# TimD1/vcfdist

Hardware: AMD Instinct MI355X
Metric: supercluster-alignments/sec (higher is better)
Workload: dtype int32; 1 GPU; wgs_synth; superclusters_per_gpu=1000000, span_dist=lognormal(median 20, sigma 1.2) clip [4,10000]

## Files before the change

### vcfdist_amd/csrc/pr_api.hip

```cpp
#include <hip/hip_runtime.h>
#include <hip/hip_ext.h>
#include <dlfcn.h>

#include <algorithm>
#include <atomic>
#include <chrono>
#include <cstdarg>
#include <cstdio>
#include <cstdlib>
#include <cstring>
#include <condition_variable>
#include <deque>
#include <functional>
#include <mutex>
#include <string>
#include <thread>
#include <tuple>
#include <unordered_map>
#include <unordered_set>
#include <vector>

#include "../../include/vcfdist_pr.h"
#include "pr_device.h"
#include "pr_plan.h"
extern "C" int vpr_batch_skeleton_from_variants(const vpr_variants *v, vpr_owned_batch **out);
#include "pr_kernels.hip"
#include "pr_band.hip"
#include "pr_walkseg.hip"
#include "pr_q16.hip"
#include "pr_zl.hip"
#include "pr_d1.hip"
#include "pr_ed.hip"
#include "pr_gen.hip"
#include "pr_wide.hip"
#include "pr_strip.hip"
#include "pr_tie.hip"

#include "pr_host.h"

namespace {


inline int plan_level_of(int lv, int long_lt, int Lt) { return (lv <= LV_Q16 && Lt >= long_lt) ? LONG_LV : lv; }

AlnDesc plan_desc(const vpr_handle *h, const Plan &P, size_t k) {
    if (!P.lazy) return P.descs[k];
    AlnDesc d = h->descs[size_t(P.work[k])];
    (void)window_layout(d, plan_level_of(P.lv, P.long_lt, d.Lt), int64_t(P.off128[k]) * 128, P.tag_or);
    return d;
}

__global__ void k_build_plan(BatchOffsets O, const int32_t *__restrict__ work, const uint32_t *__restrict__ off128, int n, int lv,
                             int long_lt, int tag_or, AlnDesc *__restrict__ plan_descs, AlnDesc *__restrict__ descs) {
    const int k = blockIdx.x * blockDim.x + threadIdx.x;
    if (k >= n) return;
    const int a = work[k];
    AlnDesc d = base_desc(O, a);
    const int dl = (lv <= LV_Q16 && d.Lt >= long_lt) ? 2  : lv;
    (void)window_layout(d, dl, int64_t(off128[k]) * 128, tag_or);
    plan_descs[k] = d;
    descs[a] = d;
}

__global__ void k_plan_keys(BatchOffsets O, int n_al, int lv, int long_lt, uint16_t *__restrict__ keys, int32_t *__restrict__ vals,
                            uint32_t *__restrict__ need) {
    const int a = blockIdx.x * blockDim.x + threadIdx.x;
    if (a >= n_al) return;
    const int sc = a >> 2, i = a & 3, qs = i >> 1, ts = 2 + (i & 1);
    AlnDesc d{};
    d.Lq = int32_t(O.hap_off[qs][sc + 1] - O.hap_off[qs][sc]);
    d.Lt = int32_t(O.hap_off[ts][sc + 1] - O.hap_off[ts][sc]);
    d.Lr = int32_t(O.ref_off[sc + 1] - O.ref_off[sc]);
    d.path_cap = d.Lq + d.Lr + d.Lt + 4;
    const int dl = (lv <= LV_Q16 && d.Lt >= long_lt) ? 2  : lv;
    keys[a] = d.Lt >= long_lt ? uint16_t(0xffff) : uint16_t(d.Lt);
    vals[a] = a;
    need[a] = uint32_t(window_layout(d, dl, 0, 0) / 128);
}
__global__ void k_plan_gather(const int32_t *__restrict__ order, const uint32_t *__restrict__ need, uint32_t *__restrict__ out,
                              int32_t *__restrict__ pos, int n) {
    const int k = blockIdx.x * blockDim.x + threadIdx.x;
    if (k >= n) return;
    const int a = order[k];
    out[k] = need[a];
    pos[a] = k;
}
__global__ void __launch_bounds__(64) k_zl_hdr(BatchOffsets O, const int32_t *__restrict__ order, int n_short, ZlWave *__restrict__ hdr) {
    const int w = blockIdx.x, lane = threadIdx.x;
    const int j = w * 64 + lane;
    int lq = 0, lr = 0, lt = 0;
    if (j < n_short) {
        const int a = order[j];
        const int sc = a >> 2, i = a & 3, qs = i >> 1, ts = 2 + (i & 1);
        lq = int32_t(O.hap_off[qs][sc + 1] - O.hap_off[qs][sc]);
        lt = int32_t(O.hap_off[ts][sc + 1] - O.hap_off[ts][sc]);
        lr = int32_t(O.ref_off[sc + 1] - O.ref_off[sc]);
    }
#pragma unroll
    for (int o = 32; o; o >>= 1) {
        lq = max(lq, __shfl_xor(lq, o)); lr = max(lr, __shfl_xor(lr, o)); lt = max(lt, __shfl_xor(lt, o));
    }
    if (lane == 0) {
        ZlWave W;
        W.in_off = 0; W.log_off = 0; W.mq = lq; W.mr = lr; W.mt = lt; W.pad = 0;
        hdr[w] = W;
    }
}
__global__ void __launch_bounds__(1024) k_zl_scan(ZlWave *__restrict__ hdr, int n_waves, int64_t *__restrict__ totals) {
    __shared__ int64_t s_in[1024], s_log[1024];
    __shared__ int s_len;
    const int tid = threadIdx.x;
    if (tid == 0) s_len = 0;
    const int per = (n_waves + 1023) / 1024;
    const int b = min(n_waves, tid * per), e = min(n_waves, b + per);
    int64_t si = 0, sl = 0;
    int lm = 0;
    for (int k = b; k < e; k++) {
        const ZlWave W = hdr[k];
        si += 64 * (int64_t(W.mq) + W.mr + W.mt); sl += 80 * int64_t(W.mt);
        lm = max(lm, max(W.mq, max(W.mr, W.mt)));
    }
    s_in[tid] = si; s_log[tid] = sl;
    __syncthreads();
    for (int o = 1; o < 1024; o <<= 1) {
        const int64_t ai = tid >= o ? s_in[tid - o] : 0, al = tid >= o ? s_log[tid - o] : 0;
        __syncthreads();
        s_in[tid] += ai; s_log[tid] += al;
        __syncthreads();
    }
    int64_t oi = s_in[tid] - si, ol = s_log[tid] - sl;
    for (int k = b; k < e; k++) {
        ZlWave W = hdr[k];
        W.in_off = oi; W.log_off = ol;
        oi += 64 * (int64_t(W.mq) + W.mr + W.mt); ol += 80 * int64_t(W.mt);
        hdr[k] = W;
    }
    if (lm) atomicMax(&s_len, lm);
    __syncthreads();
    if (tid == 1023) { totals[0] = s_in[1023]; totals[1] = s_log[1023]; totals[2] = s_len; }
}


int class_of(int len) {
    for (int k = 0; k < N_CLASSES; k++)
        if (len <= CLASSES[k].max_len) return k;
    return -1;
}

size_t fwd_lds_bytes(int cls, int Lq, int Lr) {
    const int C = CLASSES[cls].c, NT = CLASSES[cls].nt;
    const size_t PQ = (Lq + C - 1) / C * C, PR = (Lr + C - 1) / C * C;
    return (PQ + PR + 8 + 2 * (NT / 64)) * 4;
}
size_t bwd_lds_bytes(int cls, int Lq, int Lr, bool s16 = false) {
    const int C = CLASSES[cls].c, NT = CLASSES[cls].nt;
    const size_t PQ = (Lq + C - 1) / C * C, PR = (Lr + C - 1) / C * C;
    const size_t FQ = (PQ + 16 + 15) & ~size_t(15), FR = (PR + 16 + 15) & ~size_t(15);
    return (((PQ + PR + 8) * (s16 ? 2 : 4) + 15) & ~size_t(15)) + 2 * (FQ + FR) + 4 * (NT / 64) * 4 + 16;
}
bool s16_ok(const AlnDesc &d) { return d.qv_end - d.qv_beg < 32000; }

bool dense_fits(const AlnDesc &d) {
    const int cls = class_of(std::max(d.Lq, d.Lr));
    if (cls < 0 || cls >= STRIP_ONLY_CLS) return false;
    return fwd_lds_bytes(cls, d.Lq, d.Lr) <= LDS_MAX &&
           (bwd_lds_bytes(cls, d.Lq, d.Lr) <= LDS_MAX || (s16_ok(d) && bwd_lds_bytes(cls, d.Lq, d.Lr, true) <= LDS_MAX));
}

typedef void (*AlnKernel)(DevBatch, const AlnDesc *, const int32_t *, uint8_t *, AlnOut *, const int32_t *);
AlnKernel fwd_kernel(int cls) {
    switch (cls) {
        case 0: return k_fwd<64, 1>;
        case 1: return k_fwd<64, 4>;
        case 2: return k_fwd<256, 4>;
        case 3: return k_fwd<256, 8>;
        case 4: return k_fwd<1024, 8>;
        case 5: return k_fwd<1024, 16>;
        default: return k_fwd<1024, 32>;
    }
}
AlnKernel bwd_kernel(int cls, bool s16 = false) {
    if (s16) {
        switch (cls) {
            case 0: return k_bwd<64, 1, true>;
            case 1: return k_bwd<64, 4, true>;
            case 2: return k_bwd<256, 4, true>;
            case 3: return k_bwd<256, 8, true>;
            case 4: return k_bwd<1024, 8, true>;
            case 5: return k_bwd<1024, 16, true>;
            default: return k_bwd<1024, 32, true>;
        }
    }
    switch (cls) {
        case 0: return k_bwd<64, 1, false>;
        case 1: return k_bwd<64, 4, false>;
        case 2: return k_bwd<256, 4, false>;
        case 3: return k_bwd<256, 8, false>;
        case 4: return k_bwd<1024, 8, false>;
        case 5: return k_bwd<1024, 16, false>;
        default: return k_bwd<1024, 32, false>;
    }
}
typedef void (*BandFwd)(DevBatch, const AlnDesc *, const int32_t *, uint8_t *, int32_t *, AlnOut *);
typedef void (*BandBwd)(DevBatch, const AlnDesc *, const int32_t *, uint8_t *, const int32_t *, AlnOut *, int);
BandFwd band_fwd_kernel(int lv) { return lv == LV_C1 ? BandFwd(k_fwd_stripe) : lv == LV_C4 ? BandFwd(k_fwd_wide<4>) : BandFwd(k_fwd_wide<16>); }
BandBwd band_bwd_kernel(int lv) { return lv == LV_C1 ? BandBwd(k_bwd_stripe) : lv == LV_C4 ? BandBwd(k_bwd_wide<4>) : BandBwd(k_bwd_wide<16>); }
const char *band_fwd_name(int lv) { return lv == LV_Z ? "k_zero_lane" : lv == LV_Q16 ? "k_fwd_q16" : lv == LV_C1 ? "k_fwd_stripe" : lv == LV_C4 ? "k_fwd_wide<4>" : "k_fwd_wide<16>"; }
const char *band_bwd_name(int lv) { return lv <= LV_Q16 ? "k_bwd_q16" : lv == LV_C1 ? "k_bwd_stripe" : lv == LV_C4 ? "k_bwd_wide<4>" : "k_bwd_wide<16>"; }

int64_t round_up(int64_t x, int64_t m) { return (x + m - 1) / m * m; }

__global__ void k_collect_fails(const int32_t *__restrict__ work, int n, const AlnOut *__restrict__ outs,
                                int32_t *__restrict__ fail_list, int32_t *__restrict__ cnt, int pad4,
                                const int32_t *__restrict__ n_dev) {
    if (n_dev) n = min(n, *n_dev);
    const int i = blockIdx.x * blockDim.x + threadIdx.x;
    const bool live = i < n;
    const int a = live ? work[i] : -1;
    const bool bad = live && a >= 0 && !outs[a].band_ok;
    const unsigned long long mbad = __ballot(bad);
    const int lane = threadIdx.x & 63, wave = threadIdx.x >> 6;
    const int npop = __popcll(mbad);
    __shared__ int wcnt[4], wbase, wtot, wpad;
    if (lane == 0) wcnt[wave] = npop;
    __syncthreads();
    if (threadIdx.x == 0) {
        const int tot = wcnt[0] + wcnt[1] + wcnt[2] + wcnt[3];
        const int totp = pad4 ? ((tot + 3) & ~3) : tot;
        wbase = totp ? atomicAdd(cnt, totp) : 0;
        wtot = tot; wpad = totp - tot;
    }
    __syncthreads();
    int base = wbase;
    for (int w = 0; w < wave; w++) base += wcnt[w];
    if (bad) fail_list[base + __popcll(mbad & ((1ull << lane) - 1ull))] = a;
    if (int(threadIdx.x) < wpad) fail_list[wbase + wtot + int(threadIdx.x)] = -1;
}

__global__ void k_fails_count(const int32_t *__restrict__ work, int n, const AlnOut *__restrict__ outs, int32_t *__restrict__ blk,
                              int pad4, const int32_t *__restrict__ n_dev) {
    if (n_dev) n = min(n, *n_dev);
    const int i = blockIdx.x * blockDim.x + threadIdx.x;
    const int a = i < n ? work[i] : -1;
    const bool bad = a >= 0 && !outs[a].band_ok;
    const int npop = __popcll(__ballot(bad));
    __shared__ int wcnt[4];
    if ((threadIdx.x & 63) == 0) wcnt[threadIdx.x >> 6] = npop;
    __syncthreads();
    if (threadIdx.x == 0) {
        const int tot = wcnt[0] + wcnt[1] + wcnt[2] + wcnt[3];
        blk[blockIdx.x] = pad4 ? ((tot + 3) & ~3) : tot;
    }
}

#define FAILS_SCAN_NT 256
__global__ void __launch_bounds__(FAILS_SCAN_NT) k_fails_scan(int32_t *__restrict__ blk, int nb, int32_t *__restrict__ cnt) {
    __shared__ int32_t s_sum[FAILS_SCAN_NT];
    const int tid = threadIdx.x;
    const int per = (nb + FAILS_SCAN_NT - 1) / FAILS_SCAN_NT;
    const int b = min(nb, tid * per), e = min(nb, b + per);
    int32_t sum = 0;
    for (int k = b; k < e; k++) sum += blk[k];
    s_sum[tid] = sum;
    __syncthreads();
    for (int o = 1; o < FAILS_SCAN_NT; o <<= 1) {
        const int32_t v = tid >= o ? s_sum[tid - o] : 0;
        __syncthreads();
        s_sum[tid] += v;
        __syncthreads();
    }
    int32_t off = s_sum[tid] - sum;
    for (int k = b; k < e; k++) { const int32_t c = blk[k]; blk[k] = off; off += c; }
    if (tid == FAILS_SCAN_NT - 1) *cnt = s_sum[FAILS_SCAN_NT - 1];
}

__global__ void k_fails_scatter(const int32_t *__restrict__ work, int n, const AlnOut *__restrict__ outs, const int32_t *__restrict__ blk,
                                int32_t *__restrict__ fail_list, int pad4, const int32_t *__restrict__ n_dev) {
    if (n_dev) n = min(n, *n_dev);
    const int i = blockIdx.x * blockDim.x + threadIdx.x;
    const int a = i < n ? work[i] : -1;
    const bool bad = a >= 0 && !outs[a].band_ok;
    const unsigned long long mbad = __ballot(bad);
    const int lane = threadIdx.x & 63, wave = threadIdx.x >> 6;
    __shared__ int wcnt[4];
    if (lane == 0) wcnt[wave] = __popcll(mbad);
    __syncthreads();
    const int tot = wcnt[0] + wcnt[1] + wcnt[2] + wcnt[3];
// ... 298 lines not shown
            }
        } else {
            int64_t used = 0;
            size_t k0 = 0;
            for (size_t k = 0; k < n; k++) {
                const int64_t need = off[k];
                if (k > k0 && used + need > cap128) {
                    Chunk ch;
                    ch.work_off = int64_t(k0); ch.count = int32_t(k - k0);
                    P.chunks.push_back(std::move(ch));
                    P.arena_used = std::max(P.arena_used, used * 128);
                    k0 = k; used = 0;
                }
                off[k] = uint32_t(used);
                used += need;
            }
            if (n > k0) {
                Chunk ch;
                ch.work_off = int64_t(k0); ch.count = int32_t(n - k0);
                P.chunks.push_back(std::move(ch));
                P.arena_used = std::max(P.arena_used, used * 128);
            }
        }
    }
    lap("pass 2 (offsets)");
    if (!P.lazy) P.descs.resize(n);
    const size_t n_ch = P.chunks.size();
    if (lv != LV_DENSE)
        for (Chunk &ch : P.chunks) {
            ch.n_long = int32_t(std::min<int64_t>(std::max<int64_t>(int64_t(n_big) - ch.work_off, 0), ch.count));
            if (lv > LV_Q16 && (ch.n_long == ch.count || ch.count < 4096)) ch.n_long = 0;
        }
    std::vector<Sums> sums(size_t(PAR_MAX) * n_ch);
    if (P.lazy && n_ch == 1) {
        par_for(n, [&](size_t b, size_t e, int) { for (size_t k = b; k < e; k++) order[k] = alns[size_t(order[k])]; });
        Sums &S = sums[0];
        const bool no_long = P.chunks[0].n_long == 0;
        for (const Sums &T : sums1)
            for (int q = 0; q < 2; q++) {
                const int part = no_long ? 1 : q;
                S.part_cells[part] += T.part_cells[q]; S.part_in[part] += T.part_in[q];
                S.part_dense[part] += T.part_dense[q]; S.part_rows[part] += T.part_rows[q];
                S.cells += T.part_cells[q]; S.in_bytes += T.part_in[q];
            }
    } else
    par_for(n, [&](size_t b, size_t e, int tid) {
        size_t ci = 0;
        while (ci + 1 < n_ch && size_t(P.chunks[ci + 1].work_off) <= b) ci++;
        for (size_t k = b; k < e; k++) {
            while (ci + 1 < n_ch && size_t(P.chunks[ci + 1].work_off) <= k) ci++;
            const size_t pos = size_t(order[k]);
            const int32_t a = alns[pos];
            order[k] = a;
            AlnDesc d;
            if (P.lazy) { d.Lq = lq[pos]; d.Lr = lr[pos]; d.Lt = lt[pos]; d.path_cap = d.Lq + d.Lr + d.Lt + 4; }
            else d = h->descs[size_t(a)];
            const int dl = level_of(d);
            const int64_t used = int64_t(off[k]) * 128;
            if (dl != LV_DENSE) {
                (void)window_layout(d, dl, used, tag_or);
            } else {
                d.band_w = 0;
                d.pitch[0] = int32_t(round_up(d.Lq, 32)); d.pitch[1] = int32_t(round_up(d.Lr, 32));
                const int64_t m0 = round_up(int64_t(d.pitch[0]) * d.Lt, 128), m1 = round_up(int64_t(d.pitch[1]) * d.Lt, 128);
                d.band_pad = LV_TAG[dl] | tag_or;
                d.mat_off[0] = used; d.mat_off[1] = used + m0;
                d.blo_off = (used + m0 + m1) / 4;
                d.path_off = (used + m0 + m1) / int64_t(sizeof(PathEnt));
            }
            const int W = LV_WINDOW[dl];
            Sums &S = sums[size_t(tid) * n_ch + ci];
            S.cells += W ? int64_t(std::min(W, d.Lq) + std::min(W, d.Lr)) * d.Lt : int64_t(d.Lq + d.Lr) * d.Lt;
            S.in_bytes += 6 * int64_t(d.Lq) + 6 * int64_t(d.Lt) + 6 * int64_t(d.Lr);
            if (lv != LV_DENSE) {
                const int part = int64_t(k) - P.chunks[ci].work_off < P.chunks[ci].n_long ? 0 : 1;
                S.part_cells[part] += int64_t(std::min(d.band_w, d.Lq) + std::min(d.band_w, d.Lr)) * d.Lt;
                S.part_in[part] += 6 * int64_t(d.Lq) + 6 * int64_t(d.Lt) + 6 * int64_t(d.Lr);
                S.part_dense[part] += int64_t(d.Lq + d.Lr) * d.Lt;
                S.part_rows[part] += d.Lt;
            }
            h->level[size_t(a)] = uint8_t(dl);
            if (!P.lazy) P.descs[k] = d;
        }
    });
    lap("pass 3 (descriptors)");
    for (size_t ci = 0; ci < n_ch; ci++)
        for (int t = 0; t < PAR_MAX; t++) {
            const Sums &S = sums[size_t(t) * n_ch + ci];
            Chunk &ch = P.chunks[ci];
            ch.cells += S.cells;
            ch.in_bytes += S.in_bytes;
            for (int q = 0; q < 2; q++) { ch.part_cells[q] += S.part_cells[q]; ch.part_in[q] += S.part_in[q]; ch.part_dense[q] += S.part_dense[q]; ch.part_rows[q] += S.part_rows[q]; }
        }
    for (Chunk &ch : P.chunks) {
        if (lv == LV_DENSE) {
            std::vector<int32_t> idx(ch.count);
            for (int32_t w = 0; w < ch.count; w++) idx[w] = w;
            auto cls_of = [&](int32_t w) { const AlnDesc &d = P.descs[ch.work_off + w]; return class_of(std::max(d.Lq, d.Lr)); };
            std::stable_sort(idx.begin(), idx.end(), [&](int32_t x, int32_t y) { return cls_of(x) < cls_of(y); });
            std::vector<int32_t> w2(ch.count);
            std::vector<AlnDesc> d2(ch.count);
            for (int32_t w = 0; w < ch.count; w++) { w2[w] = P.work[ch.work_off + idx[w]]; d2[w] = P.descs[ch.work_off + idx[w]]; }
            std::copy(w2.begin(), w2.end(), P.work.begin() + ch.work_off);
            std::copy(d2.begin(), d2.end(), P.descs.begin() + ch.work_off);
            int32_t w = 0;
            while (w < ch.count) {
                const int c = cls_of(w);
                int32_t e = w;
                while (e < ch.count && class_of(std::max(P.descs[ch.work_off + e].Lq, P.descs[ch.work_off + e].Lr)) == c) e++;
                ch.launches.push_back(Launch{c, ch.work_off + w, e - w});
                w = e;
            }
        }
    }
    return VPR_OK;
}


int zl_finish(vpr_handle *h, size_t n_waves, int64_t in_words, int64_t log_max, int64_t in_chunk_max, int64_t n_short_max, int32_t len_max);

int prep_zero_lane(vpr_handle *h) {
    const Plan &P = h->plan0;
    std::vector<ZlWave> &hdr = h->zl_hdr_host;
    hdr.clear();
    h->zl_wave0.assign(P.chunks.size(), 0);
    int64_t in_words = 0, log_max = 0, in_chunk_max = 0, n_short_max = 0;
    int32_t len_max = 0;
    for (size_t ci = 0; ci < P.chunks.size(); ci++) {
        const Chunk &ch = P.chunks[ci];
        h->zl_wave0[ci] = int64_t(hdr.size());
        const int64_t first = ch.work_off + ch.n_long, n_short = ch.count - ch.n_long;
        const int64_t in_words0 = in_words;
        n_short_max = std::max(n_short_max, n_short);
        const size_t w0 = hdr.size(), nw = size_t((n_short + 63) / 64);
        hdr.resize(w0 + nw);
        par_for(nw * 64, [&](size_t b0, size_t e0, int) {
            for (size_t wv = (b0 + 63) / 64; wv * 64 < e0; wv++) {
                ZlWave W;
                memset(&W, 0, sizeof(W));
                for (int64_t j = int64_t(wv) * 64; j < std::min<int64_t>(n_short, int64_t(wv) * 64 + 64); j++) {
                    int32_t Lq, Lr, Lt;
                    h->descs.lens(size_t(P.work[size_t(first + j)]), Lq, Lr, Lt);
                    W.mq = std::max(W.mq, Lq); W.mr = std::max(W.mr, Lr); W.mt = std::max(W.mt, Lt);
                }
                hdr[w0 + wv] = W;
            }
        });
        int64_t log_cur = 0;
        for (size_t wv = 0; wv < nw; wv++) {
            ZlWave &W = hdr[w0 + wv];
            W.in_off = in_words;
            W.log_off = log_cur;
            in_words += 64 * (int64_t(W.mq) + W.mr + W.mt);
            log_cur += 80 * int64_t(W.mt);
            len_max = std::max(len_max, std::max(W.mq, std::max(W.mr, W.mt)));
        }
        log_max = std::max(log_max, log_cur);
        in_chunk_max = std::max(in_chunk_max, in_words - in_words0);
    }
    if (hdr.empty()) return VPR_OK;
    int rc;
    if ((rc = dev_alloc(h, &h->d_zl_hdr, hdr.size()))) return rc;
    HIPCHK(h, hipMemcpyAsync(h->d_zl_hdr, hdr.data(), hdr.size() * sizeof(ZlWave), hipMemcpyHostToDevice, h->stream));
    return zl_finish(h, hdr.size(), in_words, log_max, in_chunk_max, n_short_max, len_max);
}

int zl_finish(vpr_handle *h, size_t n_waves, int64_t in_words, int64_t log_max, int64_t in_chunk_max, int64_t n_short_max, int32_t len_max) {
    const Plan &P = h->plan0;
    int rc;
    if ((rc = dev_alloc(h, &h->d_zl_in, size_t(in_words)))) return rc;
    if ((rc = dev_alloc(h, &h->d_zl_log, size_t(log_max)))) return rc;
    if (!getenv("VPR_NO_D1")) {
        if (const char *e = getenv("VPR_D1_MAX_ROWS")) h->d1_max_rows = std::max(2, atoi(e));
        const double D1_SHARE = 0.4;
        const int64_t D1_FLOOR = int64_t(4) << 20;
        const int64_t slack = 64 * 5 * int64_t(len_max + 1);
        const int64_t in_all = 2 * in_chunk_max + slack, log_all = 2 * log_max + 160 * int64_t((n_short_max + 63) / 64) + 160 * int64_t(len_max + 1);
        h->d1_in_cap = std::min(in_all, std::max(int64_t(D1_SHARE * double(in_all)), D1_FLOOR + slack));
        h->d1_log_cap = std::min(log_all, std::max(int64_t(D1_SHARE * double(log_all)), D1_FLOOR + slack));
        const int64_t cap_ip = std::min<int64_t>(n_short_max, std::max<int64_t>(4096, (n_short_max / 4 + 3) & ~int64_t(3)));
        h->d1_wave_cap = int32_t((cap_ip + 63) / 64);
        h->d1_fail_cap = int32_t(n_short_max + n_short_max / 8 + 1024);
        h->soft_alloc = true;
        rc = dev_alloc(h, &h->d_d1_hdr, size_t(h->d1_wave_cap));
        if (!rc) rc = dev_alloc(h, &h->d_d1_in, size_t(h->d1_in_cap));
        if (!rc) rc = dev_alloc(h, &h->d_d1_log, size_t(h->d1_log_cap));
        if (!rc) rc = dev_alloc(h, &h->d_d1_fail, size_t(h->d1_fail_cap));
        if (!rc) rc = dev_alloc(h, &h->d_d1_info, 16);
        if (!rc) rc = dev_alloc(h, &h->d_d1_blk, size_t(h->d1_fail_cap / 256 + 8));
        h->soft_alloc = false;
        if (rc) {
            if (h->debug) fprintf(stderr, "[vpr] distance-1 lane level: no room for its blocks (%.2f GB), the level is off for this batch\n",
                                  double(h->d1_in_cap) * 4e-9 + double(h->d1_log_cap) * 16e-9);
            h->d_d1_hdr = nullptr; h->d_d1_in = nullptr; h->d_d1_log = nullptr; h->d_d1_fail = nullptr; h->d_d1_info = nullptr; h->d_d1_blk = nullptr;
            h->err.clear();
            (void)hipGetLastError();
        } else {
            HIPCHK(h, hipMemsetAsync(h->d_d1_info, 0, 64, h->stream));
        }
    }
    for (size_t ci = 0; ci < P.chunks.size(); ci++) {
        const Chunk &ch = P.chunks[ci];
        const int64_t n_short = ch.count - ch.n_long;
        if (n_short <= 0) continue;
        hipLaunchKernelGGL(k_prep_zl, dim3(unsigned((n_short + 63) / 64)), dim3(256), 0, h->stream, h->dB, h->d_descs,
                           P.d_work + ch.work_off + ch.n_long, int(n_short), h->d_zl_hdr + h->zl_wave0[ci], h->d_zl_in);
    }
    HIPCHK(h, hipGetLastError());
    if (h->debug) fprintf(stderr, "[vpr] zero-distance lane level: %zu waves, %.2f GB position words, %.2f GB log\n", n_waves,
                          double(in_words) * 4e-9, double(log_max) * 16e-9);
    return VPR_OK;
}

}

namespace {
int plan0_device(vpr_handle *h, int lv0, hipEvent_t ev_off, bool *done) {
    *done = false;
    const size_t na = h->descs.size();
    if (na == 0 || na > size_t(0x7fffff00) || lv0 > LV_Q16) return VPR_OK;
    Plan &P = h->plan0;
    const int LLT = h->long_lt;
    const int64_t cap128 = h->arena_bytes / 128;
    if (!h->p0.valid) return VPR_OK;
    const vpr_handle::Plan0Pass &S0 = h->p0;
    const int64_t total = S0.need128;
    if (S0.bad || S0.need_max > h->arena_bytes || total > cap128 || total > int64_t(0xfffffff0)) {
        h->level.assign(na, uint8_t(LV_DENSE));
        return VPR_OK;
    }
    std::vector<std::pair<int64_t, int32_t>> big = S0.big;
    std::sort(big.begin(), big.end());
    const size_t n = na, n_big = big.size(), n_short = n - n_big;
    {
        std::vector<int32_t> kw; std::vector<uint32_t> ko;
        kw.swap(P.work); ko.swap(P.off128);
        P = Plan();
        P.work.swap(kw); P.off128.swap(ko);
    }
    P.lv = lv0; P.arena = h->d_arena; P.tag_or = 0; P.long_lt = LLT; P.lazy = true;
    P.total_need = total * 128; P.arena_used = total * 128;
    {
        Chunk ch;
        ch.work_off = 0; ch.count = int32_t(n);
        ch.n_long = int32_t(std::min<size_t>(n_big, n));
        const bool no_long = ch.n_long == 0;
        for (int q = 0; q < 2; q++) {
            const int part = no_long ? 1 : q;
            ch.part_cells[part] += S0.part_cells[q]; ch.part_in[part] += S0.part_in[q];
            ch.part_dense[part] += S0.part_dense[q]; ch.part_rows[part] += S0.part_rows[q];
            ch.cells += S0.part_cells[q]; ch.in_bytes += S0.part_in[q];
        }
        P.chunks.push_back(std::move(ch));
    }
    int rc;
    hipStream_t ps = h->cls_stream[0];
    uint16_t *d_key = nullptr, *d_key2 = nullptr;
    int32_t *d_val = nullptr, *d_pos = nullptr;
    uint32_t *d_need = nullptr, *d_need2 = nullptr, *d_off = nullptr;
    int64_t *d_tot = nullptr;
    if ((rc = dev_alloc(h, &P.d_descs, n))) return rc;
    if ((rc = dev_alloc(h, &P.d_work, n))) return rc;
    if ((rc = dev_alloc(h, &d_key, n))) return rc;
    if ((rc = dev_alloc(h, &d_key2, n))) return rc;
    if ((rc = dev_alloc(h, &d_val, n))) return rc;
    if ((rc = dev_alloc(h, &d_pos, n))) return rc;
    if ((rc = dev_alloc(h, &d_need, n))) return rc;
    if ((rc = dev_alloc(h, &d_need2, n))) return rc;
    if ((rc = dev_alloc(h, &d_off, n))) return rc;
    if ((rc = dev_alloc(h, &d_tot, 4))) return rc;
    size_t tmp_sort = 0, tmp_scan = 0;
    if (vplan_sort_pairs_desc(nullptr, &tmp_sort, d_key, d_key2, d_val, P.d_work, n, ps) != 0 ||
        vplan_exclusive_scan_u32(nullptr, &tmp_scan, d_need2, d_off, n, ps) != 0)
        return fail(h, VPR_ERR_DEVICE, "device planner: workspace query failed");
    uint8_t *d_tmp = nullptr;
    if ((rc = dev_alloc(h, &d_tmp, std::max(tmp_sort, tmp_scan) + 256))) return rc;
    void *pin = nullptr;
    { int rc_pin = pin_alloc(h, &pin, n * 12 + n_big * 4 + 64); if (rc_pin) return rc_pin; }
    int32_t *hp_work = static_cast<int32_t *>(pin);
    uint32_t *hp_off = reinterpret_cast<uint32_t *>(hp_work + n);
    int32_t *hp_pos = reinterpret_cast<int32_t *>(hp_off + n);
    int32_t *hp_big = hp_pos + n;
    int64_t *hp_tot = reinterpret_cast<int64_t *>((reinterpret_cast<uintptr_t>(hp_big + n_big) + 15) & ~uintptr_t(15));
    for (size_t k = 0; k < n_big; k++) hp_big[k] = big[k].second;
    BatchOffsets DO;
    for (int s_ = 0; s_ < 4; s_++) { DO.hap_off[s_] = h->dB.hap_off[s_]; DO.var_off[s_] = h->dB.var_off[s_]; }
    DO.ref_off = h->dB.ref_off;
    auto blocks = [](int64_t n_) { return dim3(unsigned((n_ + 255) / 256)); };
    HIPCHK(h, hipStreamWaitEvent(ps, ev_off, 0));
    hipLaunchKernelGGL(k_plan_keys, blocks(int64_t(n)), dim3(256), 0, ps, DO, int(n), lv0, LLT, d_key, d_val, d_need);
    if (vplan_sort_pairs_desc(d_tmp, &tmp_sort, d_key, d_key2, d_val, P.d_work, n, ps) != 0) return fail(h, VPR_ERR_DEVICE, "device planner: sort failed");
    if (n_big) HIPCHK(h, hipMemcpyAsync(P.d_work, hp_big, n_big * 4, hipMemcpyHostToDevice, ps));
    hipLaunchKernelGGL(k_plan_gather, blocks(int64_t(n)), dim3(256), 0, ps, P.d_work, d_need, d_need2, d_pos, int(n));
    if (vplan_exclusive_scan_u32(d_tmp, &tmp_scan, d_need2, d_off, n, ps) != 0) return fail(h, VPR_ERR_DEVICE, "device planner: scan failed");
    HIPCHK(h, hipMemcpyAsync(hp_work, P.d_work, n * 4, hipMemcpyDeviceToHost, ps));
    HIPCHK(h, hipMemcpyAsync(hp_off, d_off, n * 4, hipMemcpyDeviceToHost, ps));
    HIPCHK(h, hipMemcpyAsync(hp_pos, d_pos, n * 4, hipMemcpyDeviceToHost, ps));
    const size_t nw = lv0 == LV_Z ? (n_short + 63) / 64 : 0;
    if (nw) {
        if ((rc = dev_alloc(h, &h->d_zl_hdr, nw))) return rc;
        hipLaunchKernelGGL(k_zl_hdr, dim3(unsigned(nw)), dim3(64), 0, ps, DO, P.d_work + n_big, int(n_short), h->d_zl_hdr);
        hipLaunchKernelGGL(k_zl_scan, dim3(1), dim3(1024), 0, ps, h->d_zl_hdr, int(nw), d_tot);
        HIPCHK(h, hipMemcpyAsync(hp_tot, d_tot, 32, hipMemcpyDeviceToHost, ps));
    }
    HIPCHK(h, hipGetLastError());
    HIPCHK(h, x_sync(h, ps, SITE));
    P.work.resize(n); P.off128.resize(n);
    h->plan0_pos.resize(na);
    par_for(n, [&](size_t b0, size_t e0, int) {
        memcpy(P.work.data() + b0, hp_work + b0, (e0 - b0) * 4);
        memcpy(P.off128.data() + b0, hp_off + b0, (e0 - b0) * 4);
        memcpy(h->plan0_pos.data() + b0, hp_pos + b0, (e0 - b0) * 4);
    });
    hipLaunchKernelGGL(k_build_plan, blocks(int64_t(n)), dim3(256), 0, h->stream, DO, P.d_work, d_off, int(n), P.lv, P.long_lt, P.tag_or,
                       P.d_descs, h->d_descs);
    if (nw) {
        h->zl_wave0.assign(1, 0);
        const int64_t in_words = hp_tot[0], log_max = hp_tot[1];
        if ((rc = zl_finish(h, nw, in_words, log_max, in_words, int64_t(n_short), int32_t(hp_tot[2])))) return rc;
    }
    *done = true;
    return VPR_OK;
}
}


extern "C" {

const char *vpr_last_error(const vpr_handle *h) { return h ? h->err.c_str() : vpr_create_error(); }

// ... 319 lines not shown
    int64_t cells = 0, bytes_alg = 0;
    {
        for (int s = 0; s < 4; s++) sec_total += 2 * b->var_off[s][n];
        sec_total += 16 * int64_t(n);
        const int lv0_ = h->cfg.band_mode == 0 ? LV_DENSE : h->cfg.band_mode == 2 ? LV_C1 : h->cfg.band_mode == 3 ? LV_Q16 : LV_Z;
        const bool plan_pass = lv0_ <= LV_Q16 && !(h->cfg.flags & VPR_CFG_HAP_DEDUP) && n > 0;
        const int LLT = h->long_lt;
        h->p0 = vpr_handle::Plan0Pass();
        if (plan_pass) h->level.resize(size_t(n) * 4);
        struct Acc { int64_t jobs = 0, cells = 0, bytes = 0; int bad = -1; vpr_handle::Plan0Pass P; };
        std::vector<Acc> acc(PAR_MAX);
        par_for(size_t(n), [&](size_t b0, size_t e0, int tid) {
            Acc &A = acc[size_t(tid)];
            AlnDesc d{};
            for (size_t scu = b0; scu < e0; scu++) {
                const int sc = int(scu);
                const int64_t Lr = b->ref_off[sc + 1] - b->ref_off[sc];
                int64_t Lh[4];
                for (int s = 0; s < 4; s++) Lh[s] = b->hap_off[s][sc + 1] - b->hap_off[s][sc];
                int64_t nv = 0;
                for (int s = 0; s < 4; s++) nv += b->var_off[s][sc + 1] - b->var_off[s][sc];
                A.bytes += 6 * (Lh[0] + Lh[1] + Lh[2] + Lh[3]) + 11 * Lr + 26 * nv;
                if ((Lh[0] < 1 || Lh[1] < 1 || Lh[2] < 1 || Lh[3] < 1 || Lr < 1) && A.bad < 0) A.bad = sc;
                for (int i = 0; i < 4; i++) {
                    const int64_t Lq = Lh[i >> 1], Lt = Lh[2 + (i & 1)];
                    A.jobs += std::min(Lr, Lt) / 33 + Lr / (ED_INLINE_LONG + 1) + Lt / (ED_INLINE_LONG + 1);
                    A.cells += (Lq + Lr) * Lt;
                    if (!plan_pass) continue;
                    d.Lq = int32_t(Lq); d.Lr = int32_t(Lr); d.Lt = int32_t(Lt);
                    d.path_cap = d.Lq + d.Lr + d.Lt + 4;
                    const int dl = plan_level_of(lv0_, LLT, d.Lt);
                    const int W = LV_WINDOW[dl], part = d.Lt >= LLT ? 0 : 1;
                    A.P.part_cells[part] += int64_t(std::min(W, d.Lq) + std::min(W, d.Lr)) * d.Lt;
                    A.P.part_in[part] += 6 * int64_t(d.Lq) + 6 * int64_t(d.Lt) + 6 * int64_t(d.Lr);
                    A.P.part_dense[part] += int64_t(d.Lq + d.Lr) * d.Lt;
                    A.P.part_rows[part] += d.Lt;
                    h->level[size_t(sc) * 4 + size_t(i)] = uint8_t(dl);
                    if (d.Lt >= LLT)
                        A.P.big.emplace_back(-(int64_t(round_up(std::min(W, d.Lq), 16) + round_up(std::min(W, d.Lr), 16)) * d.Lt), int32_t(sc * 4 + i));
                    const int64_t need = window_layout(d, dl, 0, 0);
                    A.P.need128 += need / 128;
                    A.P.need_max = std::max(A.P.need_max, need);
                    if ((d.Lt < LLT && d.Lt > 0xfffe) || d.Lq < 1 || d.Lr < 1 || d.Lt < 1) A.P.bad = true;
                }
            }
        });
        int bad = -1;
        for (const Acc &A : acc) {
            jobs_total += A.jobs; cells += A.cells; bytes_alg += A.bytes;
            if (A.bad >= 0 && (bad < 0 || A.bad < bad)) bad = A.bad;
            for (int q = 0; q < 2; q++) {
                h->p0.part_cells[q] += A.P.part_cells[q]; h->p0.part_in[q] += A.P.part_in[q];
                h->p0.part_dense[q] += A.P.part_dense[q]; h->p0.part_rows[q] += A.P.part_rows[q];
            }
            h->p0.need128 += A.P.need128; h->p0.need_max = std::max(h->p0.need_max, A.P.need_max);
            h->p0.bad = h->p0.bad || A.P.bad;
            h->p0.big.insert(h->p0.big.end(), A.P.big.begin(), A.P.big.end());
        }
        h->p0.valid = plan_pass;
        if (bad >= 0) return fail(h, VPR_ERR_ARG, "supercluster %d has an empty string", bad);
    }
    bytes_alg += 2 * cells;
    h->timing.cells_dense = cells;
    h->timing.bytes_algorithmic = bytes_alg;

    lap("descriptors");
    const size_t na = h->descs.size();
    if ((rc = dev_alloc(h, &h->d_descs, na))) return rc;
    if ((rc = dev_alloc(h, &h->d_outs, na))) return rc;
    h->n_secs_cap = sec_total;
    if ((rc = dev_alloc(h, &h->d_secs, size_t(sec_total)))) return rc;
    for (int q = 0; q < 4; q++)
        if ((rc = dev_alloc(h, &h->d_fp[q], size_t(h->n_var[q >> 1])))) return rc;
    if ((rc = dev_alloc(h, &h->d_fp_table, 4))) return rc;
    HIPCHK(h, hipMemcpyAsync(h->d_fp_table, h->d_fp, sizeof(h->d_fp), hipMemcpyHostToDevice, h->stream));
    h->jobs_cap = int32_t(std::min<int64_t>(jobs_total + 1, 0x7fffffff));
    if ((rc = dev_alloc(h, &h->d_jobs, size_t(h->jobs_cap)))) return rc;
    if ((rc = dev_alloc(h, &h->d_njobs, 1))) return rc;
    DevResults &R = h->dR;
    memset(&R, 0, sizeof(R));
    for (int s = 0; s < 4; s++) {
        const float *vq = nullptr;
        if ((rc = dev_upload(h, &vq, b->var_qual[s], size_t(h->n_var[s])))) return rc;
        R.var_qual[s] = vq;
    }
    {
        uint8_t *base = nullptr;
        size_t off = 0;
        auto place = [&](auto *&p, size_t cnt) {
            using T = std::remove_reference_t<decltype(*p)>;
            if (base) p = reinterpret_cast<T *>(base + off);
            off += (std::max<size_t>(cnt, 1) * sizeof(T) + 255) & ~size_t(255);
        };
        for (int pass = 0; pass < 2; pass++) {
            off = 0;
            for (int s = 0; s < 4; s++)
                for (int w = 0; w < 2; w++) {
                    const size_t nv = size_t(h->n_var[s]);
                    place(R.v[s][w].errtype, nv); place(R.v[s][w].sync_group, nv); place(R.v[s][w].credit, nv);
                    place(R.v[s][w].ref_ed, nv); place(R.v[s][w].query_ed, nv); place(R.v[s][w].callq, nv);
                }
            place(R.aln_dist, na); place(R.aln_end_plane, na); place(R.aln_beg_plane, na); place(R.aln_status, na);
            place(R.sc_phase, size_t(n)); place(R.orig_phase_dist, size_t(n)); place(R.swap_phase_dist, size_t(n));
            if (pass == 0) {
                if ((rc = dev_alloc(h, &base, off))) return rc;
                h->res_dev = base; h->res_bytes = off;
            }
        }
    }
    if ((rc = dev_alloc(h, &R.tally, 6))) return rc;
    R.max_qual = h->cfg.max_qual;
    R.credit_threshold = h->cfg.credit_threshold;
    R.phase_threshold = h->cfg.phase_threshold;
    h->tie_list_cap = int32_t(std::min<size_t>(std::max<size_t>(na, 4096), size_t(1) << 20));
    if ((rc = dev_alloc(h, &h->d_tie_list, size_t(h->tie_list_cap)))) return rc;
    if ((rc = dev_alloc(h, &h->d_tie_cnt, 8))) return rc;
    if ((rc = dev_alloc(h, &h->d_tie_ndec, TIE_DEC_SLOTS))) return rc;
    const size_t n_fail = 4 * na + na / 16 + 1024, n_slots = 2 + 4 * LadderCtx::N_SLOTS;
    if ((rc = dev_alloc(h, &h->d_fail, n_fail))) return rc;
    if ((rc = dev_alloc(h, &h->d_cnt, n_slots))) return rc;
    {
        void *pf = nullptr, *pc = nullptr, *pl = nullptr, *pt = nullptr;
        { int rc_pin = pin_alloc(h, &pf, n_fail * sizeof(int32_t)); if (rc_pin) return rc_pin; }
        { int rc_pin = pin_alloc(h, &pc, n_slots * sizeof(int32_t)); if (rc_pin) return rc_pin; }
        { int rc_pin = pin_alloc(h, &pl, size_t(h->tie_list_cap) * sizeof(int4)); if (rc_pin) return rc_pin; }
        { int rc_pin = pin_alloc(h, &pt, 32 * sizeof(int32_t)); if (rc_pin) return rc_pin; }
        h->hp_fail = static_cast<int32_t *>(pf);
        h->hp_cnt = static_cast<int32_t *>(pc);
        h->hp_tie_list = static_cast<int4 *>(pl);
        h->hp_tie_cnt = static_cast<int32_t *>(pt);
        h->hp_flag = h->hp_tie_cnt + 8;
        memset(h->hp_cnt, 0, n_slots * sizeof(int32_t));
        memset(h->hp_tie_cnt, 0, 32 * sizeof(int32_t));
    }

    lap("result/aux allocations");
    size_t free_b = 0, total_b = 0;
    HIPCHK(h, hipMemGetInfo(&free_b, &total_b));
    {
        const int64_t fb = books_free(int64_t(free_b), int64_t(total_b));
        if (h->debug && fb != int64_t(free_b)) fprintf(stderr, "[vpr] memory plan: the driver reports %.1f GB free, the books %.1f\n", double(free_b) / 1e9, double(fb) / 1e9);
        free_b = size_t(fb);
    }
    int64_t avail = int64_t(free_b), avail_cache = 0;
    for (const auto &c : h->dev_cache) avail_cache += int64_t(c.bytes);
    avail += avail_cache;
    int64_t scratch_kept = 0;
    for (int k = 0; k < 4; k++) for (int e = 0; e < 2; e++) scratch_kept += h->lad[k].tie_scratch_bytes[e];
    avail += scratch_kept;
    h->mem_reserve = int64_t(double(total_b) * free_share());
    avail = std::max<int64_t>(avail - h->mem_reserve, avail / 2);
    int64_t lane_est = 0;
    if (h->p0.valid && h->cfg.band_mode != 0 && h->cfg.band_mode != 2) {
        const double zl = 1.15 * (double(h->p0.part_in[1]) / 6.0 * 4.0 + 20.0 * double(h->p0.part_rows[1]));
        lane_est = int64_t(zl * (getenv("VPR_NO_D1") ? 1.0 : 1.8)) + 28 * int64_t(h->descs.size());
        avail = std::max<int64_t>(avail - lane_est, avail / 2);
    }
    int64_t budget = h->cfg.workspace_bytes > 0 ? h->cfg.workspace_bytes : int64_t(double(avail) * arena_share());
    if (budget < (8 << 20)) budget = 8 << 20;
    int64_t want = 0;
    {
        const int bm = h->cfg.band_mode;
        const bool q16ok = (bm == 1 || bm == 3);
        std::vector<int64_t> wants(PAR_MAX, 0);
        if (h->p0.valid) wants[0] = h->p0.need128 * 128 + 4096;
        else
        par_for(h->descs.size(), [&](size_t b0, size_t e0, int tid) {
          int64_t want = 0;
          for (size_t k = b0; k < e0; k++) {
            const AlnDesc &d = h->descs[k];
            int64_t flags;
            if (bm != 0 && q16ok && d.Lt < h->long_lt) {
                const int64_t nstr = (int64_t(d.Lt) + 3) / 4;
                flags = nstr * 128 + round_up(nstr * 8, 64);
            } else if (bm != 0) {
                const int W = (q16ok && bm != 2) ? LV_WINDOW[LONG_LV] : 64;
                flags = round_up(round_up(std::min(W, d.Lq), 16) * int64_t(d.Lt), 64) +
                        round_up(round_up(std::min(W, d.Lr), 16) * int64_t(d.Lt), 64) + round_up(8 * int64_t(d.Lt), 64);
            } else {
                flags = round_up(round_up(d.Lq, 32) * int64_t(d.Lt), 64) + round_up(round_up(d.Lr, 32) * int64_t(d.Lt), 64);
            }
            want += flags + round_up(int64_t(d.path_cap) * int64_t(sizeof(PathEnt)) + 128, 128) + 256;
          }
          wants[size_t(tid)] = want;
        });
        for (int64_t w : wants) want += w;
        if (h->cfg.workspace_bytes <= 0) budget = std::min(budget, std::max<int64_t>(want, 256 << 20));
    }
    h->arena_bytes = budget;
    if ((rc = dev_alloc(h, &h->d_arena, size_t(budget) + 256))) return rc;
    {
        const int64_t rest = std::max<int64_t>(avail - budget, 0);
        h->lad_budget = rest / 2; h->tie_budget = rest - rest / 2;
        h->lad_bytes = 0; h->tie_bytes = scratch_kept;
        h->want0 = want;
        int64_t first[4] = {0, 0, 0, 0}, first_sum = 0;
        for (int k = 0; k < 4; k++) {
            int64_t b2 = std::min<int64_t>(h->lad_budget / 4, int64_t(ladder_share() * double(std::max<int64_t>(want / 16, int64_t(1) << 30))));
            if (k & 1) b2 = std::min<int64_t>(b2, int64_t(2) << 30);
            first[k] = std::max<int64_t>(b2, std::min<int64_t>(int64_t(h->lad_hw[k] * double(want)), h->lad_arena_max));
            first_sum += first[k];
        }
        const double shrink = first_sum > h->lad_budget && first_sum > 0 ? double(h->lad_budget) / double(first_sum) : 1.0;
        if (h->debug)
            fprintf(stderr, "[vpr] memory plan: free %.1f GB + kept blocks %.1f + scratches %.1f, reserve %.1f, lane levels %.1f -> %.1f to plan; round 0 wants %.1f, gets %.1f; "
                            "ladders' half %.1f (first workspaces %.1f %.1f %.1f %.1f), replays' half %.1f\n",
                    double(free_b) / 1e9, double(avail_cache) / 1e9, double(scratch_kept) / 1e9, double(h->mem_reserve) / 1e9, double(lane_est) / 1e9, double(avail) / 1e9,
                    double(want) / 1e9, double(budget) / 1e9, double(h->lad_budget) / 1e9, double(first[0]) * shrink / 1e9, double(first[1]) * shrink / 1e9,
                    double(first[2]) * shrink / 1e9, double(first[3]) * shrink / 1e9, double(h->tie_budget) / 1e9);
        for (int k = (h->cfg.band_mode != 0 ? 0 : 2); k < 4; k++) {
            int64_t b2 = h->cfg.workspace_bytes;
            if (b2 <= 0) b2 = int64_t(double(first[k]) * shrink);
            if (b2 < (8 << 20)) b2 = 8 << 20;
            h->lad[k].arena_bytes = b2;
            h->lad_bytes += b2;
            if ((rc = dev_alloc(h, &h->lad[k].arena, size_t(b2) + 256))) return rc;
        }
    }

    lap("arena allocation");
    std::vector<int32_t> &all = h->scratch_i32[1];
    all.resize(na);
    h->alias.assign(size_t(b->n_sc), 0);
    h->n_aliased = 0;
    if ((rc = dev_alloc(h, &h->d_alias, size_t(std::max(b->n_sc, 1))))) return rc;
    HIPCHK(h, hipMemsetAsync(h->d_alias, 0, size_t(std::max(b->n_sc, 1)), h->stream));
    if (b->n_sc && (h->cfg.flags & VPR_CFG_HAP_DEDUP)) {
        hipLaunchKernelGGL(k_hap_alias, blocks(int64_t(b->n_sc)), dim3(256), 0, h->stream, D, h->d_alias);
        HIPCHK(h, hipMemcpyAsync(h->alias.data(), h->d_alias, size_t(b->n_sc), hipMemcpyDeviceToHost, h->stream));
        HIPCHK(h, x_sync(h, h->stream, SITE));
        size_t np = 0;
        for (size_t a = 0; a < na; a++)
            if (alias_source(h->alias[a >> 2], int(a & 3)) < 0) all[np++] = int32_t(a);
        h->n_aliased = int64_t(na - np);
        all.resize(np);
    } else {
        par_for(na, [&](size_t b0, size_t e0, int) { for (size_t k = b0; k < e0; k++) all[k] = int32_t(k); });
    }
    const size_t np = all.size();
    if (!h->p0.valid) h->level.assign(na, uint8_t(LV_DENSE));
    const int lv0 = h->cfg.band_mode == 0 ? LV_DENSE
                    : h->cfg.band_mode == 2 ? LV_C1
                    : h->cfg.band_mode == 3 ? LV_Q16 : LV_Z;
    bool dev_plan = false;
    if (np == na && lv0 <= LV_Q16 && !getenv("VPR_HOST_PLAN") && (rc = plan0_device(h, lv0, h->ev_offsets, &dev_plan))) return rc;
    if (!dev_plan && (rc = make_plan(h, all, lv0, h->plan0, h->d_arena, h->arena_bytes, 0, true))) return rc;
    lap(dev_plan ? "plan on the device" : "make_plan");
    h->d_save = nullptr; h->save_bytes = 0;
    if (lv0 <= LV_Q16 && LONG_LV == LV_C1 && !h->no_flag_save && !h->plan0.off128.empty()) {
        int64_t need = 0;
        for (const Chunk &ch : h->plan0.chunks)
            if (ch.n_long > 0)
                need = std::max<int64_t>(need, ch.n_long < ch.count ? int64_t(h->plan0.off128[size_t(ch.work_off + ch.n_long)]) * 128 : h->plan0.arena_used);
        if (need > 0 && need <= (int64_t(1) << 30)) {
            h->soft_alloc = true;
            const int rc_save = dev_alloc(h, &h->d_save, size_t(need) + 256);
            h->soft_alloc = false;
            if (rc_save == VPR_OK) h->save_bytes = need;
            else { h->d_save = nullptr; h->err.clear(); (void)hipGetLastError(); }
        }
    }
    h->level0 = h->level;
    if (!dev_plan) {
        h->plan0_pos.assign(na, -1);
        par_for(np, [&](size_t b0, size_t e0, int) { for (size_t k = b0; k < e0; k++) h->plan0_pos[size_t(h->plan0.work[k])] = int32_t(k); });
        if ((rc = dev_alloc(h, &h->plan0.d_descs, np))) return rc;
        if ((rc = dev_alloc(h, &h->plan0.d_work, np))) return rc;
    }
    lap("plan0_pos");
    if (h->n_aliased) {
        BatchOffsets DO;
        for (int s = 0; s < 4; s++) { DO.hap_off[s] = D.hap_off[s]; DO.var_off[s] = D.var_off[s]; }
        DO.ref_off = D.ref_off;
        hipLaunchKernelGGL(k_alias_descs, blocks(int64_t(na)), dim3(256), 0, h->stream, DO, h->d_alias, b->n_sc, h->d_descs);
    }
    if (dev_plan) {
    } else if (np && h->plan0.lazy) {
        void *pw = nullptr;
        { int rc_pin = pin_alloc(h, &pw, np * 8); if (rc_pin) return rc_pin; }
        int32_t *hw = static_cast<int32_t *>(pw);
        uint32_t *ho = reinterpret_cast<uint32_t *>(hw + np);
        const Plan &P0 = h->plan0;
        par_for(np, [&](size_t b0, size_t e0, int) {
            memcpy(hw + b0, P0.work.data() + b0, (e0 - b0) * 4);
            memcpy(ho + b0, P0.off128.data() + b0, (e0 - b0) * 4);
        });
        uint32_t *d_off = nullptr;
        if ((rc = dev_alloc(h, &d_off, np))) return rc;
        HIPCHK(h, hipMemcpyAsync(h->plan0.d_work, hw, np * 4, hipMemcpyHostToDevice, h->stream));
        HIPCHK(h, hipMemcpyAsync(d_off, ho, np * 4, hipMemcpyHostToDevice, h->stream));
        BatchOffsets DO;
        for (int s = 0; s < 4; s++) { DO.hap_off[s] = D.hap_off[s]; DO.var_off[s] = D.var_off[s]; }
        DO.ref_off = D.ref_off;
        hipLaunchKernelGGL(k_build_plan, blocks(int64_t(np)), dim3(256), 0, h->stream, DO, h->plan0.d_work, d_off, int(np), P0.lv,
                           P0.long_lt, P0.tag_or, h->plan0.d_descs, h->d_descs);
    } else if (np) {
        HIPCHK(h, hipMemcpyAsync(h->plan0.d_descs, h->plan0.descs.data(), np * sizeof(AlnDesc), hipMemcpyHostToDevice, h->stream));
        HIPCHK(h, hipMemcpyAsync(h->plan0.d_work, h->plan0.work.data(), np * 4, hipMemcpyHostToDevice, h->stream));
        hipLaunchKernelGGL(k_scatter_descs, blocks(int64_t(np)), dim3(256), 0, h->stream, h->plan0.d_descs, int(np), h->d_descs);
    }
    if (lv0 == LV_Z && !dev_plan && (rc = prep_zero_lane(h))) return rc;

    HIPCHK(h, x_sync(h, h->stream, SITE));
    HIPCHK(h, hipGetLastError());
    lap("plan + upload");
    uint32_t err = 0;
    HIPCHK(h, hipMemcpy(&err, h->d_err, 4, hipMemcpyDeviceToHost));
    h->n_limit_sc = err ? 1 : 0;
// ... 532 lines not shown
                    hipLaunchKernelGGL(k_fwd_strip, dim3(G.grid), dim3(ST_NT), 0, ks, h->dB, h->d_descs, d_work + g_off, g_cnt, G.d_base,
                                       G.d_tab, G.d_n, G.d_order, G.d_boff, G.d_bnd, G.d_prog, P.arena, h->d_outs, (from_window && !getenv("VPR_NO_UB")) ? 1 : 0);
                });
                if (rc) return rc;
                n_fwd++;
                vpr_launch_stat l2;
                for (const Launch &L : ch.launches) {
                    if (L.cls < STRIP_CLS) continue;
                    const KernelClass &K = CLASSES[L.cls];
                    const ClsLds Z = cls_lds(L);
                    memset(&l2, 0, sizeof(l2));
                    l2.threads = K.nt; l2.cells_per_thread = K.c; l2.n_units = L.count;
                    rc = timed(1, l2, ks, fwd_name(K).c_str(), [&] {
                        if (Z.any)
                            hipLaunchKernelGGL(fwd_kernel(L.cls), dim3(L.count), dim3(K.nt), Z.f, ks, h->dB, h->d_descs,
                                               d_work + L.work_off, P.arena, h->d_outs, G.d_ok + (L.work_off - G.off));
                        hipLaunchKernelGGL(k_fwd_finish, dim3((L.count + 255) / 256), dim3(256), 0, ks,
                                           d_work + L.work_off, L.count, h->d_outs, tag_or);
                    });
                    if (rc) return rc;
                }
                if (tag_or && ((rc = tie_replay(P, G.off, G.cnt, ks, false)) || (rc = tie_patch(P, ks, tag_or)))) return rc;
                rc = timed(2, ls, ks, "k_bwd_strip", [&] {
                    hipLaunchKernelGGL(k_bwd_strip, dim3(G.cnt), dim3(ST_NT), 0, ks, h->dB, h->d_descs, d_work + G.off, G.cnt, G.d_base,
                                       G.d_tab, G.d_n, G.d_boff, G.d_bbnd, G.d_prog + G.grid, P.arena, h->d_outs);
                });
                if (rc) return rc;
                for (const Launch &L : ch.launches) {
                    if (L.cls < STRIP_CLS) continue;
                    const KernelClass &K = CLASSES[L.cls];
                    const ClsLds Z = cls_lds(L);
                    if (!Z.any) continue;
                    memset(&l2, 0, sizeof(l2));
                    l2.threads = K.nt; l2.cells_per_thread = K.c; l2.n_units = L.count;
                    rc = timed(2, l2, ks, bwd_name(K, Z.s16).c_str(), [&] {
                        hipLaunchKernelGGL(bwd_kernel(L.cls, Z.s16), dim3(L.count), dim3(K.nt), Z.b, ks, h->dB, h->d_descs,
                                           d_work + L.work_off, P.arena, h->d_outs, G.d_ok + (L.work_off - G.off));
                    });
                    if (rc) return rc;
                }
                if ((rc = walk_launch(P, d_work + G.off, G.cnt, ks, G.cnt < 2048, tag_or))) return rc;
                if (!one_stream) {
                    HIPCHK(h, hipEventRecord(h->ev_join[STRIP_CLS], ks));
                    HIPCHK(h, hipStreamWaitEvent(base, h->ev_join[STRIP_CLS], 0));
                }
            }
        }
        return VPR_OK;
    }

    int enqueue_part(const Plan &P, const int32_t *d_work, int64_t off, int32_t cnt, int lv, hipStream_t ks,
                            int slot, int64_t fail_off, bool long_part, int64_t part_cells, int64_t part_in,
                            int64_t part_dense, int dtag_override = -1, int phases = 7,
                            const int32_t *n_dev = nullptr, int32_t n_all = 0, int tag_or = 0) {
        const int W = LV_WINDOW[lv], C = W / 64, tag = LV_TAG[lv] | tag_or;
        const bool q16 = lv <= LV_Q16, zero = lv == LV_Z;
        const int dtag = dtag_override >= 0 ? dtag_override : tag;
        const int32_t *list = d_work + off;
        int32_t *a_i32 = reinterpret_cast<int32_t *>(P.arena);
        PathEnt *a_path = reinterpret_cast<PathEnt *>(P.arena);
        vpr_launch_stat ls;
        memset(&ls, 0, sizeof(ls));
        ls.threads = q16 ? 16 : 64; ls.cells_per_thread = q16 ? 1 : C; ls.n_units = cnt;
        ls.cells = part_cells;
        ls.cells_dense = part_dense;
        ls.bytes_algorithmic = ls.cells + part_in;
        int rc = VPR_OK;
        if (phases & 1) {
        if (zero) {
            ls.bytes_algorithmic = 36 * zl_rows;
            ls.cells = 8 * zl_rows;
        }
        cells_touched += ls.cells;
        const bool save = lv == LV_C1 && !tag_or && fwd_save_delta != 0;
        RestoreJob *rjobs = nullptr;
        bool restore = false;
        if (lv == LV_C1 && tag_or && h->d_save && tie_resident && !n_dev) {
            void *pb = nullptr;
            { int rc_pin = exec_pin(h, &pb, size_t(cnt) * sizeof(RestoreJob)); if (rc_pin) return rc_pin; }
            rjobs = static_cast<RestoreJob *>(pb);
            restore = true;
            for (int32_t k = 0; k < cnt && restore; k++) {
                const auto it = tie_early.find(P.work[size_t(off) + size_t(k)]);
                if (it == tie_early.end() || it->second.plan != &h->plan0 || (it->second.mode != 1 && it->second.mode != 3) ||
                    it->second.pos < tie_resident->work_off || it->second.pos >= tie_resident->work_off + tie_resident->n_long) { restore = false; break; }
                const AlnDesc od = plan_desc(h, h->plan0, size_t(it->second.pos)), nd = plan_desc(h, P, size_t(off) + size_t(k));
                if (od.band_pad != LV_TAG[LV_C1] || od.pitch[0] != nd.pitch[0] || od.pitch[1] != nd.pitch[1] ||
                    od.mat_off[1] + int64_t(od.pitch[1]) * od.Lt > h->save_bytes) { restore = false; break; }
                rjobs[k] = RestoreJob{{od.mat_off[0], od.mat_off[1]}, od.blo_off};
            }
        }
        rc = timed(1, ls, ks, restore ? "k_restore_stripe" : band_fwd_name(lv), [&] {
            if (zero)
                hipExtLaunchKernelGGL(k_zero_lane, dim3((cnt + 63) / 64), dim3(64), h->zl_lds_bytes, ks, own_a, own_b, 0, h->d_descs, list, cnt,
                                      h->d_zl_hdr + zl_wave0, h->d_zl_in, h->d_zl_log, h->d_outs, a_path,
                                      (h->cfg.flags & VPR_CFG_KEEP_PATHS) ? 1 : 0, h->d_d1_hdr ? h->d1_max_rows : 0, h->lane_prio_rows);
            else if (q16)
                hipLaunchKernelGGL(k_fwd_q16, dim3((cnt + 3) / 4), dim3(64), 0, ks, h->dB, h->d_descs, list, cnt,
                                   P.arena, a_i32, h->d_outs, n_dev);
            else if (restore)
                hipLaunchKernelGGL(k_restore_stripe, dim3(cnt), dim3(256), 0, ks, h->d_descs, list, rjobs, h->plan0.arena,
                                   int64_t(reinterpret_cast<intptr_t>(h->d_save) - reinterpret_cast<intptr_t>(h->plan0.arena)), P.arena, a_i32);
            else if (save)
                hipLaunchKernelGGL(k_fwd_stripe_save, dim3(cnt), dim3(64), 0, ks, h->dB, h->d_descs, list, P.arena, a_i32, h->d_outs,
                                   fwd_save_delta);
            else
                hipLaunchKernelGGL(band_fwd_kernel(lv), dim3(cnt), dim3(lv >= LV_C4 ? W : 64), 0,
                                   ks, h->dB, h->d_descs, list, P.arena, a_i32, h->d_outs);
            hipLaunchKernelGGL(k_fwd_band_finish, dim3((cnt + 255) / 256), dim3(256), 0, ks, list, cnt, h->d_outs, tag, n_dev);
        }, zero);
        if (rc) return rc;
        n_fwd++;
        {
            const int32_t nc = n_dev ? n_all : cnt;
            if (zero && h->d_d1_blk) ordered_fails(list, nc, h->d_fail + fail_off, h->d_cnt + slot, n_dev, ks);
            else
            hipLaunchKernelGGL(k_collect_fails, dim3((nc + 255) / 256), dim3(256), 0, ks, list, nc, h->d_outs,
                               h->d_fail + fail_off, h->d_cnt + slot, zero ? 1 : 0, n_dev);
            hipLaunchKernelGGL(k_publish_fails, dim3(zero ? 1 : std::min((nc + 255) / 256, 1024)), dim3(256), 0, ks,
                               h->d_fail + fail_off, h->d_cnt + slot, h->hp_fail + fail_off, h->hp_cnt + slot, zero ? 0 : 1);
        }
        HIPCHK(h, hipEventRecord(h->ev_slot[slot], ks));
        }
        if ((phases & 2) && !zero) {
        ls.bytes_algorithmic = ls.cells;
        rc = timed(2, ls, ks, band_bwd_name(lv), [&] {
            if (q16)
                hipLaunchKernelGGL(k_bwd_q16, dim3((cnt + 3) / 4), dim3(64), 0, ks, h->dB, h->d_descs, list, cnt,
                                   P.arena, a_i32, h->d_outs, tag, dtag, n_dev);
            else
                hipLaunchKernelGGL(band_bwd_kernel(lv), dim3(cnt), dim3(lv >= LV_C4 ? W : 64), 0,
                                   ks, h->dB, h->d_descs, list, P.arena, a_i32, h->d_outs, tag);
        });
        if (rc) return rc;
        }
        if (!(phases & 4)) return rc;
        const bool wave_walk = !q16 && (long_part || cnt < 2048);
        int64_t walk_rows_sum = 0;
        if (lv == LV_C1 && !h->seq_walk)
            for (int32_t k = 0; k < cnt && walk_rows_sum <= WSEG_MAX_ROWS; k++) walk_rows_sum += plan_desc(h, P, size_t(off) + size_t(k)).Lt;
        const bool seg_walk = lv == LV_C1 && !h->seq_walk && walk_rows_sum <= WSEG_MAX_ROWS;
        const bool row_walk = lv == LV_C1 && (wave_walk || seg_walk);
        vpr_launch_stat ws_;
        memset(&ws_, 0, sizeof(ws_));
        ws_.threads = q16 ? 16 : 64; ws_.n_units = cnt; ws_.cells_per_thread = 2;
        if (q16) {
            if (!zero) rc = timed(3, ws_, ks, "k_walk_q16", [&] {
                hipLaunchKernelGGL(k_walk_q16, dim3((cnt + 3) / 4), dim3(64), 0, ks, h->dB, h->d_descs, list, cnt,
                                   P.arena, a_i32, h->d_outs, a_path, tag, dtag, n_dev);
            });
            if (rc) return rc;
            ws_.cells_per_thread = 3;
            if (zero) {
                ws_.bytes_algorithmic = 20 * zl_rows;
                rc = timed(3, ws_, ks, "k_zero_walk", [&] {
                    hipLaunchKernelGGL(k_zero_walk, dim3((cnt + 63) / 64), dim3(64), 0, ks, h->d_descs, list, cnt, h->d_zl_hdr + zl_wave0,
                                       h->d_zl_in, h->d_zl_log, h->d_outs, a_path, (h->cfg.flags & VPR_CFG_KEEP_PATHS) ? 1 : 0, tag,
                                       h->lane_prio_rows);
                });
                if (rc) return rc;
                ws_.bytes_algorithmic = 0;
            }
            if (zero) rc = timed(3, ws_, ks, "k_zero_credit", [&] {
                hipLaunchKernelGGL(k_zero_credit, dim3((cnt + 63) / 64), dim3(64), 0, ks, h->dB, h->d_descs, list, cnt,
                                   h->d_zl_hdr + zl_wave0, h->d_zl_log, h->d_outs, h->d_secs, h->d_fp_table, h->d_jobs,
                                   h->d_njobs, h->jobs_cap, tag);
            });
            else if (cnt <= CREDIT_WAVE_MAX && !n_dev) rc = timed(3, ws_, ks, "k_credit<wave>", [&] {
                hipLaunchKernelGGL(k_credit<true>, dim3(cnt), dim3(64), 0, ks, h->dB, h->d_descs, list, cnt,
                                   h->d_outs, a_path, h->d_secs, h->d_fp_table, h->d_jobs, h->d_njobs,
                                   h->jobs_cap, dtag, tag, n_dev);
            });
            else {
                static const int head_max = [] { const char *e = exp_getenv("VPR_CREDIT_HEAD"); return e ? atoi(e) : 4096; }();
                const int32_t head = (n_dev && h->d_d1_blk && cnt > 2 * head_max) ? head_max : 0;
                if (head > 0) {
                    vpr_launch_stat wh_ = ws_;
                    wh_.n_units = head;
                    rc = timed(3, wh_, ks, "k_credit<wave>", [&] {
                        hipLaunchKernelGGL(k_credit<true>, dim3(head), dim3(64), 0, ks, h->dB, h->d_descs, list, head,
                                           h->d_outs, a_path, h->d_secs, h->d_fp_table, h->d_jobs, h->d_njobs,
                                           h->jobs_cap, dtag, tag, n_dev, 0);
                    });
                    if (rc) return rc;
                }
                rc = timed(3, ws_, ks, "k_credit<lane>", [&] {
                    hipLaunchKernelGGL(k_credit<false>, dim3((cnt - head + 63) / 64), dim3(64), 0, ks, h->dB, h->d_descs,
                                       list, cnt, h->d_outs, a_path, h->d_secs, h->d_fp_table, h->d_jobs,
                                       h->d_njobs, h->jobs_cap, dtag, tag, n_dev, int(head));
                });
            }
        } else if (row_walk) {
            static const int wseg_min_rows = [] { const char *e = exp_getenv("VPR_WSEG_MIN_ROWS"); return e ? atoi(e) : 2048; }();
            int32_t n_seg = cnt;
            if (seg_walk && long_part && wseg_min_rows > 0) {
                n_seg = 0;
                while (n_seg < cnt && plan_desc(h, P, size_t(off) + size_t(n_seg)).Lt >= wseg_min_rows) n_seg++;
            }
            if (!seg_walk || n_seg < cnt) {
                const int32_t k0 = seg_walk ? n_seg : 0;
                vpr_launch_stat wr_ = ws_;
                wr_.n_units = cnt - k0;
                rc = timed(3, wr_, ks, "k_walk_rows", [&] {
                    hipLaunchKernelGGL(k_walk_rows, dim3(cnt - k0), dim3(64), 0, ks, h->dB, h->d_descs, list + k0, cnt - k0,
                                       P.arena, a_i32, h->d_outs, a_path, tag);
                });
                if (rc) return rc;
            }
            if (seg_walk && n_seg > 0) {
                const int32_t cnt_all = cnt;
                const int32_t cnt = n_seg;
                (void)cnt_all;
                int64_t rows_sum = 0;
                for (int32_t k = 0; k < cnt; k++) rows_sum += plan_desc(h, P, size_t(off) + size_t(k)).Lt;
                ws_.n_units = cnt;
                WsegTables T;
                T.cap = int32_t(std::min<int64_t>(rows_sum / WSEG_ROWS + cnt + 1, 0x7fffffff));
                void *q = nullptr;
                const size_t b_cnt = 256, b_base = round_up(int64_t(cnt) * 4, 256), b_own = round_up(int64_t(T.cap) * 8, 256),
                             b_map = size_t(T.cap) * 128 * 8, b_ent = size_t(T.cap) * 16;
                if ((rc = exec_alloc(h, &q, b_cnt + b_base + b_own + b_map + b_ent))) return rc;
                uint8_t *u = static_cast<uint8_t *>(q);
                T.counter = reinterpret_cast<int32_t *>(u); u += b_cnt;
                T.seg_base = reinterpret_cast<int32_t *>(u); u += b_base;
                T.owner = reinterpret_cast<int2 *>(u); u += b_own;
                T.map = reinterpret_cast<uint2 *>(u); u += b_map;
                T.entry = reinterpret_cast<int4 *>(u);
                HIPCHK(h, hipMemsetAsync(T.counter, 0, 4, ks));
                rc = timed(3, ws_, ks, "k_walk_seg", [&] {
                    hipLaunchKernelGGL(k_wseg_plan, blocks(cnt), dim3(256), 0, ks, h->d_descs, list, cnt, h->d_outs, tag, T);
                    hipLaunchKernelGGL(k_wseg_map, dim3(T.cap), dim3(128), 0, ks, h->dB, h->d_descs, list, P.arena, a_i32, T);
                    hipLaunchKernelGGL(k_wseg_compose, dim3(cnt), dim3(64), 0, ks, h->d_descs, list, cnt, a_i32, h->d_outs, T);
                    hipLaunchKernelGGL(k_wseg_emit, dim3(T.cap), dim3(64), 0, ks, h->dB, h->d_descs, list, P.arena, a_i32, h->d_outs,
                                       a_path, T);
                });
            }
            if (rc) return rc;
            ws_.cells_per_thread = 3;
            ws_.n_units = cnt;
            const bool wave_credit = wave_walk || cnt <= CREDIT_WAVE_MAX;
            rc = timed(3, ws_, ks, wave_credit ? "k_credit<wave>" : "k_credit<lane>", [&] {
                if (wave_credit)
                    hipLaunchKernelGGL(k_credit<true>, dim3(cnt), dim3(64), 0, ks, h->dB, h->d_descs, list, cnt,
                                       h->d_outs, a_path, h->d_secs, h->d_fp_table, h->d_jobs, h->d_njobs,
                                       h->jobs_cap, dtag, tag, n_dev);
                else
                    hipLaunchKernelGGL(k_credit<false>, dim3((cnt + 63) / 64), dim3(64), 0, ks, h->dB, h->d_descs,
                                       list, cnt, h->d_outs, a_path, h->d_secs, h->d_fp_table, h->d_jobs,
                                       h->d_njobs, h->jobs_cap, dtag, tag, n_dev);
            });
        } else {
            rc = walk_launch(P, list, cnt, ks, wave_walk, tag);
        }
        return rc;
    }

    void ordered_fails(const int32_t *list, int32_t nc, int32_t *out, int32_t *cnt, const int32_t *n_dev, hipStream_t ks) {
        const int nb = (nc + 255) / 256;
        hipLaunchKernelGGL(k_fails_count, dim3(nb), dim3(256), 0, ks, list, nc, h->d_outs, h->d_d1_blk, 1, n_dev);
        hipLaunchKernelGGL(k_fails_scan, dim3(1), dim3(FAILS_SCAN_NT), 0, ks, h->d_d1_blk, nb, cnt);
        hipLaunchKernelGGL(k_fails_scatter, dim3(nb), dim3(256), 0, ks, list, nc, h->d_outs, h->d_d1_blk, out, 1, n_dev);
    }

    int enqueue_d1(const int32_t *list, const int32_t *n_dev, int32_t cap, int32_t n_all, hipStream_t ks, int ph, int ztag) {
        const int nw = (cap + 63) / 64;
        vpr_launch_stat ls;
        memset(&ls, 0, sizeof(ls));
        ls.threads = 64; ls.cells_per_thread = 1; ls.n_units = cap;
        int rc = VPR_OK;
        if (ph == 1) {
            rc = timed(0, ls, ks, "k_prep_d1", [&] {
                hipLaunchKernelGGL(k_d1_hdr, dim3(nw), dim3(64), 0, ks, h->d_descs, list, n_dev, cap, h->d_outs, h->d_d1_hdr);
                hipLaunchKernelGGL(k_d1_scan, dim3(1), dim3(D1_SCAN_NT), 0, ks, h->d_d1_hdr, nw, h->d1_in_cap, h->d1_log_cap, h->d_d1_info);
                hipLaunchKernelGGL(k_prep_d1, dim3(nw), dim3(256), 0, ks, h->dB, h->d_descs, list, n_dev, cap, h->d_outs, h->d_d1_hdr, h->d_d1_in);
            });
            if (rc) return rc;
            rc = timed(1, ls, ks, "k_one_lane", [&] {
                hipLaunchKernelGGL(k_one_lane, dim3(nw), dim3(64), 0, ks, h->d_descs, list, n_dev, cap, h->d_d1_hdr, h->d_d1_in, h->d_d1_log,
                                   h->d_outs, reinterpret_cast<PathEnt *>(h->plan0.arena), (h->cfg.flags & VPR_CFG_KEEP_PATHS) ? 1 : 0, h->d_d1_info,
                                   std::max(1, h->lane_prio_rows / 4));
                hipLaunchKernelGGL(k_fwd_band_finish, dim3((cap + 255) / 256), dim3(256), 0, ks, list, cap, h->d_outs, D1_TAG, n_dev);
            });
            if (rc) return rc;
            ordered_fails(list, n_all, h->d_d1_fail, h->d_d1_info + 2, n_dev, ks);
        } else if (ph == 4) {
            ls.cells_per_thread = 3;
            rc = timed(3, ls, ks, "k_one_walk", [&] {
                hipLaunchKernelGGL(k_one_walk, dim3(nw), dim3(64), 0, ks, h->d_descs, list, n_dev, cap, h->d_d1_hdr, h->d_d1_in, h->d_d1_log,
                                   h->d_outs, reinterpret_cast<PathEnt *>(h->plan0.arena), (h->cfg.flags & VPR_CFG_KEEP_PATHS) ? 1 : 0, h->d_d1_info,
                                   std::max(1, h->lane_prio_rows / 4));
            });
            if (rc) return rc;
            rc = timed(3, ls, ks, "k_one_credit", [&] {
                hipLaunchKernelGGL(k_one_credit, dim3(nw), dim3(64), 0, ks, h->dB, h->d_descs, list, n_dev, cap, h->d_d1_hdr, h->d_d1_log,
                                   h->d_outs, h->d_secs, h->d_fp_table, h->d_jobs, h->d_njobs, h->jobs_cap, ztag);
            });
        }
        return rc;
    }

    int read_fails(int slot, int64_t fail_off, hipStream_t ls, std::vector<int32_t> &fails) {
        HIPCHK(h, x_event_sync(h, h->ev_slot[slot], SITE));
        const int32_t nf = h->hp_cnt[slot];
        if (nf > 0) {
            const size_t f0 = fails.size();
            fails.insert(fails.end(), h->hp_fail + fail_off, h->hp_fail + fail_off + nf);
            if (h->debug && nf <= (getenv("VPR_DEBUG_REJECTS") ? atoi(getenv("VPR_DEBUG_REJECTS")) : 64)) {
                for (size_t k = f0; k < fails.size(); k++) {
                    const int32_t a = fails[k];
                    AlnOut o;
                    (void)hipMemcpyAsync(&o, h->d_outs + a, sizeof(o), hipMemcpyDeviceToHost, ls);
                    (void)x_sync(h, ls, SITE);
                    const AlnDesc &d = h->descs[a];
                    fprintf(stderr, "[vpr] level %d rejected sc %d aln %d: Lq %d Lr %d Lt %d  s %d exit_min %d dq %d dr %d\n",
                            int(h->level[a]), d.sc, d.aln, d.Lq, d.Lr, d.Lt, o.s, o.exit_min, o.dist_q, o.dist_r);
                }
            }
        }
        return VPR_OK;
    }

    bool overlap(const LadderCtx &c) const { return !h->no_round_overlap && !h->no_strips && c.ls2 != nullptr && (&c - h->lad) < 2; }
    int lad_sync(LadderCtx &c) {
        HIPCHK(h, x_sync(h, c.ls, SITE));
        if (overlap(c)) HIPCHK(h, x_sync(h, c.ls2, SITE));
        return VPR_OK;
    }
    int lad_flush(LadderCtx &c, std::vector<int32_t> &out) {
        for (const auto &pd : c.pending) {
            int rc = read_fails(pd.first, pd.second, c.ls, out);
            if (rc) return rc;
        }
        c.pending.clear();
        c.plans.clear();
        c.slot_cur = 0; c.fail_cur = 0;
        if (!overlap(c)) { c.stage_cur = 0; c.arena_cur = 0; }
        return VPR_OK;
    }

    int lad_tie_off(int k) { return h->tie_list_cap / 2 + k * (h->tie_list_cap / 4); }

    int lad_tie_cap(int k) { (void)k; return h->tie_list_cap / 4; }

    void ladder_collect(int k, const int32_t *list, int32_t n, hipStream_t ks) {
        hipLaunchKernelGGL(k_collect_ties_list, blocks(n), dim3(256), 0, ks, list, n, h->d_outs, h->d_tie_list + lad_tie_off(k),
                           h->d_tie_cnt + 5 + k, lad_tie_cap(k));
        hipLaunchKernelGGL(k_publish_ties, dim3(4), dim3(256), 0, ks, h->d_tie_list + lad_tie_off(k), h->d_tie_cnt + 5 + k,
                           h->hp_tie_list + lad_tie_off(k), h->hp_tie_cnt + 5 + k, lad_tie_cap(k));
        post_flag(9 + k, ks);
        lad_tie_wait[k] = true;
    }

    void drop_resident(const LadderCtx &c) {
        for (auto &r : h->resident)
            if (r.second >= c.arena && r.second < c.arena + c.arena_bytes) r.second = nullptr;
    }

    bool lad_grow(LadderCtx &c, int64_t nb, int64_t must = 0) {
        const int k = int(&c - h->lad);
        for (int j = 0; j < 4; j++) {
            LadderCtx &g = h->lad[j];
            const bool sibling = &g != &c;
            if (sibling && !(k < 2 && j == 1 - k)) continue;
            if (g.arena_bytes >= nb) continue;
            const int64_t need = sibling ? 0 : must;
            int64_t nb_g = std::max<int64_t>(std::min<int64_t>(nb, h->lad_budget - h->lad_bytes), need);
            if (nb_g < g.arena_bytes + g.arena_bytes / 2 && need <= g.arena_bytes) {
                if (!sibling) return false;
                continue;
            }
            uint8_t *na2 = nullptr;
            h->soft_alloc = true;
            int rc_grow = dev_alloc(h, &na2, size_t(nb_g) + 256);
            h->soft_alloc = false;
            if (rc_grow != VPR_OK && need > g.arena_bytes && need < nb_g) {
                h->err.clear();
                (void)hipGetLastError();
                nb_g = need;
                rc_grow = dev_alloc(h, &na2, size_t(nb_g) + 256);
            }
            if (rc_grow != VPR_OK) {
                h->err.clear();
                (void)hipGetLastError();
                if (!sibling) return false;
                continue;
            }
            h->lad_bytes += nb_g;
            g.arena = na2; g.arena_bytes = nb_g; g.arena_cur = 0;
        }
        return true;
    }

    int lad_start(LadderCtx &c, std::vector<int32_t> &fails, std::vector<int32_t> &carry, bool tie = false) {
        if (fails.empty()) return VPR_OK;
        if (!tie) n_retry += int64_t(fails.size());
        std::sort(fails.begin(), fails.end());
        std::vector<int32_t> by_lv[LV_DENSE + 1];
        for (int32_t a : fails) by_lv[std::min<int>(tie ? std::max<int>(h->level[size_t(a)], LV_Q16) : h->level[size_t(a)] + 1, LV_DENSE)].push_back(a);
        if (h->debug)
            fprintf(stderr, "[vpr] retry round (ladder %d): %zu -> 16, %zu -> 64, %zu -> 256, %zu -> 1024, %zu -> dense\n",
                    int(&c - h->lad), by_lv[1].size(), by_lv[2].size(), by_lv[3].size(), by_lv[4].size(), by_lv[5].size());
        const size_t nf = fails.size();
        if (c.work_cap < c.stage_cur + nf || c.hp_cap < c.stage_cur + nf) {
            const int k = int(&c - h->lad);
            for (int j = 0; j < 4; j++) {
                LadderCtx &g = h->lad[j];
                if (&g != &c && !(k < 2 && j == 1 - k)) continue;
                const size_t cap = std::max<size_t>(2 * (c.stage_cur + nf), 1 << 14);
                if (g.work_cap >= cap && g.hp_cap >= cap && &g != &c) continue;
                void *pd = nullptr, *pw = nullptr;
                int32_t *dw_ = nullptr;
                int rc = dev_alloc(h, &dw_, cap);
                if (rc) return rc;
                { int rc_pin = pin_alloc(h, &pd, cap * sizeof(AlnDesc)); if (rc_pin) return rc_pin; }
                { int rc_pin = pin_alloc(h, &pw, cap * sizeof(int32_t)); if (rc_pin) return rc_pin; }
                g.d_work = dw_; g.work_cap = cap;
                g.hp_descs = static_cast<AlnDesc *>(pd); g.hp_work = static_cast<int32_t *>(pw); g.hp_cap = cap;
                g.stage_cur = 0;
            }
        }
        bool zero_slots = true;
        std::vector<std::function<int()>> later;
        c.plans.reserve(c.plans.size() + LV_DENSE + 1);
        if (c.arena_cur == 0) drop_resident(c);
        if (!tie) hipLaunchKernelGGL(k_flag, dim3(1), dim3(1), 0, c.ls, h->d_tie_cnt + 5 + int(&c - h->lad), 0);
        for (int lv = LV_Q16; lv <= LV_DENSE; lv++) {
            if (by_lv[lv].empty()) continue;
            c.plans.emplace_back();
            Plan &P = c.plans.back();
            const int tag_or = tie ? TIE_TAG_BIT : 0;
            trace("    level %d: %zu alignments, planning", lv, by_lv[lv].size());
            int rc = make_plan(h, by_lv[lv], lv, P, c.arena + c.arena_cur, c.arena_bytes - c.arena_cur, tag_or);
            trace("    planned");
            if (rc == VPR_OK && P.chunks.size() > 1 && c.arena_cur > 0) rc = VPR_ERR_NOMEM;
            if (rc == VPR_ERR_NOMEM && c.arena_cur > 0) {
                { const int rs = lad_sync(c); if (rs) return rs; }
                c.arena_cur = 0;
                drop_resident(c);
                rc = make_plan(h, by_lv[lv], lv, P, c.arena, c.arena_bytes, tag_or);
            }
            if (rc == VPR_OK && P.chunks.size() > 1 && h->cfg.workspace_bytes <= 0) {
                const int64_t nb = std::min<int64_t>((overlap(c) ? 2 : 1) * P.total_need + (1 << 20), h->lad_arena_max);
                if (nb > c.arena_bytes + c.arena_bytes / 2 && lad_grow(c, nb))
                    rc = make_plan(h, by_lv[lv], lv, P, c.arena, c.arena_bytes, tag_or);
            }
            if (rc == VPR_ERR_NOMEM && h->cfg.workspace_bytes <= 0) {
                if (lad_grow(c, std::max<int64_t>(2 * h->last_need, 2 * c.arena_bytes), h->last_need + (1 << 20)))
                    rc = make_plan(h, by_lv[lv], lv, P, c.arena, c.arena_bytes, tag_or);
// ... 779 lines not shown
```

### vcfdist_amd/csrc/pr_d1.hip

```cpp
#ifndef PR_D1_HIP_
#define PR_D1_HIP_

#define D1_TAG 9
#define D1_CLEAN ZL_CLEAN_REJECT

#define GE_ALIVE 1u
#define GE_MAT 2u
#define GE_SWP 4u
#define GE_PSLOT_SHIFT 3
#define GE_SUB 32u
#define GE_SUB_SHIFT 6
#define GE_INS 256u
#define GE_INS_SHIFT 9
#define GE_DEL 2048u
#define GE_DEL_SHIFT 12
#define GE_TP 16384u
#define GE_BWD 32768u

#define MV_SWP_R 0
#define MV_MAT 1
#define MV_SUB 2
#define MV_INS 3
#define MV_DEL 4
#define MV_SWP_Q 5
// ... 452 lines not shown
#pragma unroll
            for (int p = 0; p < 2; p++) upper = upper || (act && (fq[p][2] >= 0 || fq[p][3] >= 0 || gq[p][2] >= 0 || gq[p][3] >= 0));
            if (__any(upper) || !fg_row(S2{}, t, act, tw1, bp)) (void)fg_row(S4{}, t, act, tw1, bp);
        }
        { const int c_ = __popcll(__ballot(ok)); if (lane == 0 && c_) atomicAdd(info + 6, c_); }
        ok = ok && gq[0][0] == Lq - 1;
        { const int c_ = __popcll(__ballot(ok)); if (lane == 0 && c_) atomicAdd(info + 7, c_); }
    }
    lapck(1);
    if (live) {
        AlnOut &o = outs[a];
        o.dist_q = ok ? 1 : D_INF;
        o.dist_r = D_INF;
        o.exit_min = ok ? D_INF : 0;
    }
    if (!__any(ok)) return;

    const int nrow = ok ? Lt : 0;
    int bmax = nrow;
#pragma unroll
    for (int o = 32; o; o >>= 1) bmax = max(bmax, __shfl_xor(bmax, o));
    int beg_plane = VPR_PLANE_REF;
    {
        int kf[2][4], kg[2][4];
        uint32_t cf[2] = {0, 0};
        uint32_t cg[2][2] = {{0, 0}, {0, 0}};
#pragma unroll
        for (int p = 0; p < 2; p++) {
#pragma unroll
            for (int s = 0; s < 4; s++) { kf[p][s] = -1; kg[p][s] = -1; }
        }
        auto key = [](int from, int tp, int rank, int slot) -> int { return (((from >> 5) + tp) << 5) | ((7 - rank) << 2) | slot; };
        auto sc_row = [&](auto Sc, int t, bool act, bool first, const zl_u2 pf, const zl_u4 pgv) {
            constexpr int S = decltype(Sc)::value;
            int bf[2][S], bg[2][S];
#pragma unroll
            for (int p = 0; p < 2; p++) {
#pragma unroll
                for (int s = 0; s < S; s++) { bf[p][s] = -1; bg[p][s] = -1; }
            }
            if (first) bg[0][0] = 0x1f;
            if (__any(act && !first)) {
#pragma unroll
                for (int p = 0; p < 2; p++) {
                    const int o = 1 - p;
#pragma unroll
                    for (int s = 0; s < S; s++) {
                        {
                            const uint32_t e = (cg[p][s >> 1] >> (16 * (s & 1))) & 0xffffu;
                            const bool on = act && !first && kg[p][s] >= 0;
                            if (__any(on)) {
                                const int tp = (e & GE_TP) ? 1 : 0;
                                if (on && (e & GE_MAT)) bg[p][s] = max(bg[p][s], key(kg[p][s], tp, MV_MAT, s));
                                const bool sw = on && (e & GE_SWP) && (e & GE_BWD);
                                const int ps = int((e >> GE_PSLOT_SHIFT) & 3u);
                                const int ksw = key(kg[p][s], p == 1 ? 0 : tp, o == 1 ? MV_SWP_R : MV_SWP_Q, s);
                                const bool su = on && (e & GE_SUB), de = on && (e & GE_DEL);
                                const int ss = int((e >> GE_SUB_SHIFT) & 3u), ds = int((e >> GE_DEL_SHIFT) & 3u);
                                const int ksu = key(kg[p][s], tp, MV_SUB, s), kde = key(kg[p][s], 0, MV_DEL, s);
#pragma unroll
                                for (int k = 0; k < S; k++) {
                                    bg[o][k] = (sw && ps == k) ? max(bg[o][k], ksw) : bg[o][k];
                                    bf[p][k] = (su && ss == k) ? max(bf[p][k], ksu) : bf[p][k];
                                    bf[p][k] = (de && ds == k) ? max(bf[p][k], kde) : bf[p][k];
                                }
                            }
                        }
                        {
                            const uint32_t e = (cf[p] >> (8 * s)) & 0xffu;
                            const bool on = act && !first && kf[p][s] >= 0;
                            if (__any(on)) {
                                const int tp = (e & ZE_TP) ? 1 : 0;
                                if (on && (e & ZE_HASMAT)) bf[p][s] = max(bf[p][s], key(kf[p][s], tp, MV_MAT, s));
                                const bool sw = on && (e & ZE_HASSWP) && (e & ZE_BWD);
                                const int ps = int((e >> ZE_PSLOT_SHIFT) & 3u);
                                const int ksw = key(kf[p][s], p == 1 ? 0 : tp, o == 1 ? MV_SWP_R : MV_SWP_Q, s);
#pragma unroll
                                for (int k = 0; k < S; k++) bf[o][k] = (sw && ps == k) ? max(bf[o][k], ksw) : bf[o][k];
                            }
                        }
                    }
                }
            }
            const uint32_t pgw[2][2] = {{pgv.x, pgv.y}, {pgv.z, pgv.w}};
#pragma unroll
            for (int p = 0; p < 2; p++) {
#pragma unroll
                for (int s = 0; s < S; s++) {
                    const uint32_t e = (pgw[p][s >> 1] >> (16 * (s & 1))) & 0xffffu;
                    const bool in = act && bg[p][s] >= 0 && (e & GE_INS);
                    if (!__any(in)) continue;
                    const int is = int((e >> GE_INS_SHIFT) & 3u);
                    const int kin = key(bg[p][s], (e & GE_TP) ? 1 : 0, MV_INS, s);
#pragma unroll
                    for (int k = 0; k < S; k++) bf[p][k] = (in && is == k) ? max(bf[p][k], kin) : bf[p][k];
                }
            }
            {
                zl_u4 mv;
                uint32_t b[4] = {0xffff0000u, 0xffff0000u, 0xffff0000u, 0xffff0000u};
                if constexpr (S == 4) { b[0] = b[1] = b[2] = b[3] = 0u; }
#pragma unroll
                for (int p = 0; p < 2; p++) {
#pragma unroll
                    for (int s = 0; s < S; s++) {
                        const uint32_t mf = bf[p][s] < 0 ? 0xffu : (uint32_t(7 - ((bf[p][s] >> 2) & 7)) | (uint32_t(bf[p][s] & 3) << 3));
                        const uint32_t mg = bg[p][s] < 0 ? 0xffu : (uint32_t(7 - ((bg[p][s] >> 2) & 7)) | (uint32_t(bg[p][s] & 3) << 3));
                        b[p] |= mf << (8 * s);
                        b[2 + p] |= mg << (8 * s);
                    }
                }
                mv.x = b[0]; mv.y = b[1]; mv.z = b[2]; mv.w = b[3];
                __builtin_amdgcn_raw_buffer_store_b128(mv, rlog, act ? (uint32_t(t) << 10) + lane16 : ZL_OOB, 0, 0);
            }
            if (act) {
#pragma unroll
                for (int p = 0; p < 2; p++) {
#pragma unroll
                    for (int s = 0; s < 4; s++) {
                        if (s < S) { kf[p][s] = bf[p][s]; kg[p][s] = bg[p][s]; }
                        else { kf[p][s] = -1; kg[p][s] = -1; }
                    }
                    cg[p][0] = pgw[p][0]; cg[p][1] = pgw[p][1];
                }
                cf[0] = pf.x; cf[1] = pf.y;
            }
        };
        auto f_row = [&](int t) -> zl_u2 { return __builtin_amdgcn_raw_buffer_load_b64(rlog, (t >= 0 && t < nrow) ? logB1 + (uint32_t(t) << 9) + lane8 : ZL_OOB, 0, 0); };
        auto g_row = [&](int t) -> zl_u4 { return __builtin_amdgcn_raw_buffer_load_b128(rlog, (t >= 0 && t < nrow) ? logB2 + (uint32_t(t) << 10) + lane16 : ZL_OOB, 0, 0); };
        zl_u2 pf_n = f_row(bmax - 1);
        zl_u4 pg_n = g_row(bmax - 1);
        for (int t = bmax - 1; t >= 0; t--) {
            const bool act = t < nrow;
            const bool first = act && t == nrow - 1;
            const zl_u2 pf = pf_n;
            const zl_u4 pgv = pg_n;
            pf_n = f_row(t - 1);
            pg_n = g_row(t - 1);
            const bool upper = act && ((((cf[0] | cf[1] | pf.x | pf.y) & 0xffff0000u) | cg[0][1] | cg[1][1] | pgv.y | pgv.w) != 0u);
#ifdef D1_CLOCKS
            if (lane == 0) { atomicAdd(info + 14, 1); if (__any(upper)) atomicAdd(info + 15, 1); }
#endif
            if (__any(upper)) sc_row(S4{}, t, act, first, pf, pgv);
            else sc_row(S2{}, t, act, first, pf, pgv);
        }
        beg_plane = kf[0][0] >= 0 ? VPR_PLANE_QUERY : VPR_PLANE_REF;
        ok = ok && (kf[0][0] >= 0 || kf[1][0] >= 0);
    }

    lapck(2);
    if (ok) { AlnOut &o = outs[a]; o.beg_plane = beg_plane; o.path_len = -1; }
}

__global__ void __launch_bounds__(64, 8) k_one_walk(const AlnDesc *__restrict__ descs, const int32_t *__restrict__ list,
                                                    const int32_t *__restrict__ n_dev, int n_cap, const ZlWave *__restrict__ hdr,
                                                    const uint32_t *__restrict__ zin, uint4 *__restrict__ zlog,
                                                    AlnOut *__restrict__ outs, PathEnt *__restrict__ paths, int keep_paths,
                                                    int32_t *__restrict__ info, int prio_rows) {
    const int w = blockIdx.x, lane = threadIdx.x;
    const ZlWave H = hdr[w];
    if (H.mt <= 0) return;
    if (H.mt >= prio_rows) __builtin_amdgcn_s_setprio(2);
    const int n_list = min(*n_dev, n_cap);
    const int wi = w * 64 + lane;
    const int a_ = wi < n_list ? list[wi] : -1;
    const int a = max(a_, 0);
    const AlnDesc *dp = descs + a;
    const bool ok = a_ >= 0 && outs[a].band_ok == D1_TAG && outs[a].path_len == -1;
    const int Lq = ok ? dp->Lq : 1, Lr = ok ? dp->Lr : 1;
    const int L[2] = {Lq, Lr};
    const int nrow = ok ? dp->Lt : 0;
    int bmax = nrow;
#pragma unroll
    for (int o = 32; o; o >>= 1) bmax = max(bmax, __shfl_xor(bmax, o));
    if (bmax == 0) return;
    const auto rin = __builtin_amdgcn_make_buffer_rsrc(const_cast<uint32_t *>(zin + H.in_off), 0, 256 * (2 * H.mq + 2 * H.mr + H.mt), 0x00020000);
    const auto rlog = __builtin_amdgcn_make_buffer_rsrc(zlog + H.log_off, 0, 2560 * (H.mt + 1), 0x00020000);
    const uint32_t lane4 = uint32_t(lane) << 2, lane8 = uint32_t(lane) << 3, lane16 = uint32_t(lane) << 4;
    const uint32_t posW[2] = {0u, uint32_t(2 * H.mq) << 8};
    const uint32_t post = uint32_t(2 * H.mq + 2 * H.mr) << 8;
    const uint32_t logB1 = uint32_t(H.mt + 1) << 10;
    auto in_at = [&](uint32_t off) -> uint32_t { return __builtin_amdgcn_raw_buffer_load_b32(rin, off, 0, 0); };
    auto word_at = [&](int p, int x, bool on) -> uint32_t { return in_at(on ? posW[p] + (uint32_t(x) << 8) + lane4 : ZL_OOB); };
    auto t_at = [&](int t, bool on) -> uint32_t { return in_at(on ? post + (uint32_t(t) << 8) + lane4 : ZL_OOB); };
    const int beg_plane = ok ? outs[a].beg_plane : 0;
    auto lapck = [&](int) {};
    {
        PathEnt *path = paths + dp->path_off;
        const uint32_t logS0 = logB1;
        int hi = beg_plane, slot = 0, layer = 0, x = 0, ti = 0, mv_in = -1;
        uint32_t status = 0;
        bool wok = ok, done = !ok;
        int plen = 0;
        for (int i = 0; i <= bmax; i++) {
            const bool act = wok && !done;
            if (!__any(act)) break;
            const uint32_t mvw = __builtin_amdgcn_raw_buffer_load_b32(rlog, act ? (uint32_t(ti) << 10) + lane16 + (uint32_t(layer) << 3) + (uint32_t(hi) << 2) : ZL_OOB, 0, 0);
            const uint32_t tw = t_at(ti, act);
            const uint32_t cw = word_at(hi, x, act);
            const int trv = ZW_PTR(tw), qref = hi ? x : ZW_PTR(cw);
            uint32_t sync = 1, edit = 0;
            if (mv_in >= 0) {
                const bool diag = mv_in != MV_INS && mv_in != MV_DEL;
                const bool in_t = (tw & ZW_PV) && !(tw & ZW_PB);
                const bool in_q = hi == 0 && (cw & ZW_PV) && !(cw & ZW_PB);
                sync = (diag && !in_t && !in_q && !((tw | cw) & ZW_INS) && trv == qref) ? 1u : 0u;
                edit = (mv_in == MV_SUB || mv_in == MV_INS || mv_in == MV_DEL) ? 1u : 0u;
            }
            const uint32_t eqb = (ZW_BASE(cw) == ZW_BASE(tw) ? 1u : 0u) | ((hi || !(cw & ZW_PV)) ? 2u : 0u);
            zl_u2 st;
            st.x = uint32_t(x) | (uint32_t(hi) << 16) | (sync << 17) | (eqb << 18) | (edit << 20) | (uint32_t(i - ti) << 21);
            st.y = uint32_t(qref + 1) | (uint32_t(trv + 1) << 16);
            __builtin_amdgcn_raw_buffer_store_b64(st, rlog, act ? logS0 + (uint32_t(i) << 9) + lane8 : ZL_OOB, 0, 0);
            if ((keep_paths & 1) && act) {
                uint4 pe;
                pe.x = uint32_t(x) | (uint32_t(hi) << 31);
                pe.y = uint32_t(ti) | (sync << 31) | (edit << 30);
                pe.z = uint32_t(qref);
                pe.w = uint32_t(trv);
                *reinterpret_cast<uint4 *>(path + i) = pe;
            }
            if (act) {
                if (layer == 1 && hi == 0 && x == Lq - 1 && ti == nrow - 1) { done = true; plen = i + 1; }
                else {
                    const uint32_t m = (mvw >> (8 * slot)) & 0xffu;
                    const int rank = int(m & 7u), to = int((m >> 3) & 3u);
                    if (m == 0xffu) { status |= VPR_ST_ERR_NO_PTR; wok = false; }
                    else if (rank == MV_MAT) { x++; ti++; }
                    else if (rank == MV_SWP_R || rank == MV_SWP_Q) { x = ZW_PTR(cw) + 1; hi = 1 - hi; slot = to; ti++; }
                    else if (rank == MV_SUB) { x++; ti++; layer = 1; slot = to; }
                    else if (rank == MV_INS) { x++; layer = 1; slot = to; }
                    else { ti++; layer = 1; slot = to; }
                    mv_in = rank;
                    if (ti >= nrow || x >= L[hi]) { status |= VPR_ST_ERR_NO_PTR; wok = false; }
                }
            }
        }
        lapck(3);
        {
            const int nf = __popcll(__ballot(ok && wok && done));
            if (lane == 0 && nf) atomicAdd(info + 4, nf);
        }
        if (ok) {
            AlnOut &o = outs[a];
            wok = wok && done;
            if (!wok) status |= VPR_ST_ERR_NO_PTR;
            o.beg_plane = beg_plane;
            o.path_len = wok ? plen : 0;
            if (!wok) o.n_sec = 0;
            if (status) atomicOr(&o.status, status);
        }
    }
}

struct D1Fetch {
    const uint2 *log;
    int64_t pre_i;
    uint2 pre;
    __device__ PathEnt operator()(int64_t i) {
        const uint2 v = (i == pre_i) ? pre : log[i * 64];
        if (i > 0) { pre_i = i - 1; pre = log[(i - 1) * 64]; }
        PathEnt e;
        e.a = (v.x & 0xffffu) | (((v.x >> 16) & 1u) << 31);
        e.b = uint32_t(i - int64_t((v.x >> 21) & 1u)) | (((v.x >> 17) & 1u) << 31) | (((v.x >> 20) & 1u) << 30) | (((v.x >> 18) & 3u) << 28);
        e.qref = int(v.y & 0xffffu) - 1;
        e.tref = int(v.y >> 16) - 1;
        return e;
    }
};

__global__ void __launch_bounds__(64) k_one_credit(DevBatch B, const AlnDesc *__restrict__ descs, const int32_t *__restrict__ list,
                                                   const int32_t *__restrict__ n_dev, int n_cap, const ZlWave *__restrict__ hdr,
                                                   const uint4 *__restrict__ zlog, AlnOut *__restrict__ outs, Section *__restrict__ secs,
                                                   int32_t *const *__restrict__ fp_group, EdJob *__restrict__ jobs,
                                                   int32_t *__restrict__ n_jobs, int32_t jobs_cap, int ztag) {
    const int w = blockIdx.x, lane = threadIdx.x;
    const ZlWave H = hdr[w];
    if (H.mt <= 0) return;
    const int wi = w * 64 + lane;
    if (wi >= min(*n_dev, n_cap)) return;
    const int a = list[wi];
    if (a < 0) return;
    const AlnDesc d = descs[a];
    AlnOut &O = outs[a];
    if (d.band_pad != ztag || O.band_ok != D1_TAG) return;
    if (O.status & (VPR_ST_ERR_NO_PTR | VPR_ST_ERR_LIMIT)) return;
    D1Fetch f{reinterpret_cast<const uint2 *>(zlog + H.log_off + 64 * (int64_t(H.mt) + 1)) + lane, -1, make_uint2(0, 0)};
    credit_walk<false, D1Fetch, true>(B, d, O, a, nullptr, int64_t(O.path_len), 0u, secs, fp_group, jobs, n_jobs, jobs_cap, true, f);
}

#endif
```

### vcfdist_amd/csrc/pr_kernels.hip

```cpp
#include <hip/hip_runtime.h>
#include <stdint.h>

#include "../../include/vcfdist_pr.h"
#include "pr_device.h"
#include "pr_scan.h"

__device__ __forceinline__ bool fwd_allow(int f) { return !(f & PV) || (f & PE); }
__device__ __forceinline__ bool bwd_allow(int f) { return !(f & PV) || (f & PB); }

__global__ void __launch_bounds__(256) k_prep_scof(DevBatch B) {
    __shared__ int64_t s_off[257];
    const int which = blockIdx.y;
    const int64_t *off = which < 4 ? B.hap_off[which] : B.ref_off;
    int32_t *out = which < 4 ? B.sc_hap[which] : B.sc_ref;
    const int sc0 = blockIdx.x * 256, m = min(256, B.n_sc - sc0);
    for (int i = threadIdx.x; i <= m; i += 256) s_off[i] = off[sc0 + i];
    __syncthreads();
    const int64_t beg = s_off[0], end = s_off[m];
    for (int64_t g = beg + threadIdx.x; g < end; g += 256) {
        int lo = 0, hi = m;
        while (hi - lo > 1) {
            const int mid = (lo + hi) >> 1;
            if (s_off[mid] <= g) lo = mid; else hi = mid;
        }
// ... 387 lines not shown
#pragma unroll
        for (int c = 0; c < C; c++) { sc[p][c] = S_NEG; f1[p][c] = 0; }
    for (int p = 0; p < 2; p++)
        if (q0 < Pp[p])
#pragma unroll
            for (int c = 0; c < C; c++) { s_st(p, q0 + c, S_NEG); FROW(0, p, q0 + c) = 0; }
    uint8_t f0[2][C];
#pragma unroll
    for (int p = 0; p < 2; p++) {
#pragma unroll
        for (int c = 0; c < C; c++) f0[p][c] = 0;
        if (q0 < Lp[p]) {
            typename FlagVec<C>::T v = *reinterpret_cast<const typename FlagVec<C>::T *>(mat[p] + size_t(Lt - 1) * d.pitch[p] + q0);
            __builtin_memcpy(f0[p], &v, C);
#pragma unroll
            for (int c = 0; c < C; c++) FROW(1, p, q0 + c) = f0[p][c];
        } else if (q0 < Pp[p]) {
#pragma unroll
            for (int c = 0; c < C; c++) FROW(1, p, q0 + c) = 0;
        }
    }
    if (tid == 0) {
        for (int p = 0; p < 2; p++) { s_st(p, Pp[p], S_NEG); FROW(0, p, Pp[p]) = 0; FROW(1, p, Pp[p]) = 0; }
    }
    lds_barrier<NT>();
    uint32_t tie_used = 0;
    FlagReg<C> pf[2];
#pragma unroll
    for (int p = 0; p < 2; p++)
        if (Lt >= 2 && q0 < Lp[p]) pf[p] = load_flags<C>(mat[p] + size_t(Lt - 2) * d.pitch[p] + q0);

    for (int t = Lt - 1; t >= 0; t--) {
        const int cur = (Lt - 1 - t + 1) & 1;
        const int nxt = cur ^ 1;

        int32_t base[2][C];
        uint8_t bm[2][C];
        int8_t lk[2][C];
        MP g[2];
#pragma unroll
        for (int p = 0; p < 2; p++) {
            const int o = 1 - p;
            int xs_r = S_NEG; int xf_r = 0, xf0_r = 0, xtp_r = 0;
            if (q0 + C <= Pp[p]) {
                xs_r = s_ld(p, q0 + C);
                xf_r = FROW(nxt, p, q0 + C);
                xf0_r = FROW(cur, p, q0 + C);
            }
            if (p == 0) xtp_r = xtp_right;
            MP G; G.A = S_NEG; G.B = 0;
            bool first = true;
#pragma unroll
            for (int c = C - 1; c >= 0; c--) {
                const int q = q0 + c;
                const int xs = (c == C - 1) ? xs_r : sc[p][c + 1];
                const int xf = (c == C - 1) ? xf_r : f1[p][c + 1];
                const int xtp = (c == C - 1) ? xtp_r : (kc[p][c + 1] & 1);
                int best = S_NEG; uint8_t m = 0;
                if (f_diag(xf)) {
                    const int v = xs + xtp;
                    best = v; m = uint8_t(f_diag(xf));
                }
                if (f1[p][c] & F_DEL) {
                    const int v = sc[p][c];
                    if (v > best) { best = v; m = F_DEL; } else if (v == best) m |= F_DEL;
                }
                if (zq[p][c] >= 0) {
                    const int zf = FROW(nxt, o, zq[p][c]);
                    if ((zf & F_SWP) && f_choice_of(zf) == rank_of(kc[p][c])) {
                        const int v = s_ld(o, zq[p][c]) + ((kc[p][c] >> 3) & 1);
                        if (v >= 0 && (zf & F_TIE)) tie_used++;
                        if (v > best) { best = v; m = F_SWP; } else if (v == best) m |= F_SWP;
                    }
                }
                if (t == Lt - 1 && p == end_plane && q == Lp[p] - 1) { best = 0; m = F_MAT; }
                if (q >= Lp[p]) { best = S_NEG; m = 0; }
                base[p][c] = best;
                bm[p][c] = m;
                const int xf0 = (c == C - 1) ? xf0_r : f0[p][c + 1];
                const int l = (xf0 & F_INS) ? xtp : -1;
                lk[p][c] = l;
                MP F; F.A = best; F.B = l;
                if (first) { G = F; first = false; } else G = mp_compose(F, G);
            }
            g[p] = G;
        }
        int inq, inr;
        block_suffix_mp2<NT>(g[0], g[1], inq, inr, wsc);
        const int inc[2] = {inq, inr};
        uint8_t out[2][C];
#pragma unroll
        for (int p = 0; p < 2; p++) {
            int prev = inc[p];
#pragma unroll
            for (int c = C - 1; c >= 0; c--) {
                int v = base[p][c];
                uint8_t m = bm[p][c];
                if (lk[p][c] >= 0) {
                    const int w = prev + lk[p][c];
                    if (w > v) { v = w; m = F_INS; } else if (w == v) m |= F_INS;
                }
                if (v < 0) { v = S_NEG; m = 0; }
                sc[p][c] = v;
                out[p][c] = m ? uint8_t(m | (f0[p][c] & F_KEEP)) : uint8_t(0);
                prev = v;
                f1[p][c] = f0[p][c];
            }
            if (q0 < Lp[p]) {
#pragma unroll
                for (int c = 0; c < C; c++) s_st(p, q0 + c, sc[p][c]);
                if (t > 0) {
                    unpack_flags<C>(pf[p], f0[p]);
#pragma unroll
                    for (int c = 0; c < C; c++) FROW(nxt, p, q0 + c) = f0[p][c];
                }
            }
        }
#pragma unroll
        for (int p = 0; p < 2; p++)
            if (t > 1 && q0 < Lp[p]) pf[p] = load_flags<C>(mat[p] + size_t(t - 2) * d.pitch[p] + q0);
#pragma unroll
        for (int p = 0; p < 2; p++)
            if (q0 < Lp[p]) {
                typename FlagVec<C>::T v;
                __builtin_memcpy(&v, out[p], C);
                *reinterpret_cast<typename FlagVec<C>::T *>(mat[p] + size_t(t) * d.pitch[p] + q0) = v;
            }
        lds_barrier<NT>();
    }
    if (tid == 0) outs[a].beg_plane = (sc[0][0] >= 0) ? VPR_PLANE_QUERY : VPR_PLANE_REF;
    if (tie_used) { atomicOr(&outs[a].status, VPR_ST_SWAP_TIE); outs[a].band_ok = TIE_MARK(0); atomicAdd(&outs[a].n_sec, int(tie_used)); }
}

#undef FROW

#define ED_INLINE_LONG 256
__device__ int small_ed(const uint8_t *a, int m, const uint8_t *b, int n) {
    int row[33];
    for (int j = 0; j <= n; j++) row[j] = j;
    for (int i = 1; i <= m; i++) {
        int diag = row[0];
        row[0] = i;
        const uint8_t ai = a[i - 1];
        for (int j = 1; j <= n; j++) {
            const int up = row[j];
            const int v = min(min(up + 1, row[j - 1] + 1), diag + (ai != b[j - 1]));
            diag = up;
            row[j] = v;
        }
    }
    return row[n];
}

struct NoFetch { __device__ PathEnt operator()(int64_t) const { return PathEnt{0, 0, 0, 0}; } };
template <bool WAVE, class XF = NoFetch, bool EXT = false>
__device__ __forceinline__ void credit_walk(const DevBatch &B, const AlnDesc &d, AlnOut &O, const int a,
                                            const PathEnt *__restrict__ path, const int64_t n, uint32_t status,
                                            Section *__restrict__ secs, int32_t *const *__restrict__ fp_group,
                                            EdJob *__restrict__ jobs, int32_t *__restrict__ n_jobs, int32_t jobs_cap,
                                            const bool lead, XF xf = XF()) {
    const int qi = 0, ri = 1;
    const int32_t *q2r = B.hap_ptr[d.qs] + d.q_off;
    const int32_t *t2r = B.hap_ptr[d.ts] + d.t_off;
    const int q_size = d.Lq, r_size = d.Lr, t_size = d.Lt;
    (void)qi;
    const uint8_t *Rs = B.ref_seq + d.r_off;
    const uint8_t *Ts = B.hap_seq[d.ts] + d.t_off;
    const int swap = (d.aln == 1 || d.aln == 2);
    const int32_t *qv_pos = B.var_pos[d.qs];
    const int32_t *tv_pos = B.var_pos[d.ts];
    int32_t *fpg = fp_group[d.qs * 2 + swap];
    Section *sec = secs + d.sec_off;
    int n_sec = 0;

    int sync_group = 0;
    const int end_hi = O.end_plane;
    int cur_hi = end_hi;
    const int qri_size = (end_hi == qi) ? q_size : r_size;
    int prev_hi = cur_hi, prev_qri = qri_size - 1, prev_ti = t_size - 1;
    int prev_qref = (end_hi == ri) ? r_size - 1 : q2r[q_size - 1];
    int prev_tref = t2r[t_size - 1];
    int prev_sync_ref_idx = r_size, prev_sync_truth_idx = t_size;
    int query_ed = 0;
    int64_t query_var_ptr = d.qv_end - 1, truth_var_ptr = d.tv_end - 1;
    int query_var_pos = (query_var_ptr >= d.qv_beg) ? qv_pos[query_var_ptr] : 0;
    int truth_var_pos = (truth_var_ptr >= d.tv_beg) ? tv_pos[truth_var_ptr] : 0;
    int64_t prev_query_var_ptr = query_var_ptr, prev_truth_var_ptr = truth_var_ptr;
    int64_t sync_idx = n;

    const int lane_ = threadIdx.x & 63;
    int64_t cbase = 0;
    PathEnt ccur = PathEnt{0, 0, 0, 0}, cpre = PathEnt{0, 0, 0, 0};
    if (WAVE) {
        cbase = (n > 0) ? ((n - 1) & ~int64_t(63)) : 0;
        if (cbase + lane_ < n) ccur = path[cbase + lane_];
        if (cbase >= 64) cpre = path[cbase - 64 + lane_];
    }
    PathEnt q0 = ccur, q1 = ccur, q2 = ccur, q3 = ccur, q4 = ccur, q5 = ccur, q6 = ccur, q7 = ccur;
    int64_t qbase = int64_t(1) << 60;
    auto fetch = [&](int64_t i) -> PathEnt {
        if constexpr (EXT) {
            return xf(i);
        } else if (WAVE) {
            if (i < cbase) {
                cbase -= 64;
                ccur = cpre;
                if (cbase >= 64) cpre = path[cbase - 64 + lane_];
            }
            const int l = int(i - cbase);
            PathEnt e;
            e.a = uint32_t(__builtin_amdgcn_readlane(int(ccur.a), l));
            e.b = uint32_t(__builtin_amdgcn_readlane(int(ccur.b), l));
            e.qref = __builtin_amdgcn_readlane(ccur.qref, l);
            e.tref = __builtin_amdgcn_readlane(ccur.tref, l);
            return e;
        } else {
            if (i < qbase) {
                qbase = i & ~int64_t(7);
                const uint4 *src = reinterpret_cast<const uint4 *>(path + qbase);
                const uint4 v0 = src[0], v1 = src[1], v2 = src[2], v3 = src[3], v4 = src[4], v5 = src[5], v6 = src[6], v7 = src[7];
                q0 = PathEnt{v0.x, v0.y, int(v0.z), int(v0.w)};
                q1 = PathEnt{v1.x, v1.y, int(v1.z), int(v1.w)};
                q2 = PathEnt{v2.x, v2.y, int(v2.z), int(v2.w)};
                q3 = PathEnt{v3.x, v3.y, int(v3.z), int(v3.w)};
                q4 = PathEnt{v4.x, v4.y, int(v4.z), int(v4.w)};
                q5 = PathEnt{v5.x, v5.y, int(v5.z), int(v5.w)};
                q6 = PathEnt{v6.x, v6.y, int(v6.z), int(v6.w)};
                q7 = PathEnt{v7.x, v7.y, int(v7.z), int(v7.w)};
            }
            const int k = int(i - qbase);
            PathEnt e = q0;
            if (k == 1) e = q1;
            if (k == 2) e = q2;
            if (k == 3) e = q3;
            if (k == 4) e = q4;
            if (k == 5) e = q5;
            if (k == 6) e = q6;
            if (k == 7) e = q7;
            return e;
        }
    };
    uint32_t cur_b = 0;
    uint32_t eq_next = 0, eq_cur = 0;
    int nx_qref = -2, nx_ti = -2;
    int rs_base = 1 << 30, ts_base = 1 << 30;
    int rs_cur = 0, ts_cur = 0;
    auto rs_at = [&](int i) -> int {
        if constexpr (WAVE) {
            if (i < rs_base || i >= rs_base + 64) {
                rs_base = max(0, i - 63);
                const int x = rs_base + lane_;
                rs_cur = x < r_size ? int(Rs[x]) : 0;
            }
            return __builtin_amdgcn_readlane(rs_cur, i - rs_base);
        } else {
            return int(Rs[i]);
        }
    };
    auto ts_at = [&](int i) -> int {
        if constexpr (WAVE) {
            if (i < ts_base || i >= ts_base + 64) {
                ts_base = max(0, i - 63);
                const int x = ts_base + lane_;
                ts_cur = x < t_size ? int(Ts[x]) : 0;
            }
            return __builtin_amdgcn_readlane(ts_cur, i - ts_base);
        } else {
            return int(Ts[i]);
        }
    };

    bool clean = false;
    int64_t pl_base = -1;
    bool pl_static = false;
    auto plain_static = [&]() {
        const int qr = ccur.qref, ti = int(ccur.b & 0x0fffffffu);
        const bool have = cbase + lane_ < n;
        const bool eqb = have && qr >= 0 && qr < r_size && ti < t_size && Rs[qr] == Ts[ti];
        const int qr_up = __shfl_down(qr, 1), ti_up = __shfl_down(ti, 1);
        const bool eq_up = __shfl_down(int(eqb), 1) != 0;
        pl_static = have && lane_ < 63 && cbase + lane_ + 1 < n && (ccur.b >> 31) && !((ccur.b >> 30) & 1u) &&
                    qr_up == qr + 1 && ti_up == ti + 1 && eq_up;
        pl_base = cbase;
    };
    while (sync_idx >= 0) {
        if constexpr (WAVE && !EXT) {
            if (clean && sync_idx < n) {
                if (pl_base != cbase) plain_static();
                const int l = int(sync_idx - cbase);
                const bool plain = pl_static && ccur.qref >= query_var_pos && ccur.tref >= truth_var_pos;
                const unsigned long long below = (l == 63) ? ~0ull : ((2ull << l) - 1ull);
                const unsigned long long stop = ~__ballot(plain) & below;
                const int run = stop ? l - (63 - __builtin_clzll(stop)) : l + 1;
                if (run > 0) {
                    const int lj = l - run + 1;
                    prev_qref = __builtin_amdgcn_readlane(ccur.qref, lj);
                    prev_tref = __builtin_amdgcn_readlane(ccur.tref, lj);
                    cur_b = uint32_t(__builtin_amdgcn_readlane(int(ccur.b), lj));
                    prev_hi = int(uint32_t(__builtin_amdgcn_readlane(int(ccur.a), lj)) >> 31);
                    prev_ti = int(cur_b & 0x0fffffffu);
                    prev_sync_ref_idx = prev_qref + 1;
                    prev_sync_truth_idx = prev_ti + 1;
                    eq_cur = (cur_b >> 28) & 3u;
                    sync_idx -= run;
                    if (sync_idx < 0) break;
                    cur_hi = prev_hi;
                    const PathEnt e = fetch(sync_idx);
                    cur_b = e.b;
                    eq_next = eq_cur; eq_cur = (e.b >> 28) & 3u;
                    nx_qref = prev_qref; nx_ti = prev_ti;
                    prev_qri = int(e.a & 0x7fffffffu);
                    prev_hi = int(e.a >> 31);
                    prev_ti = int(e.b & 0x0fffffffu);
                    prev_qref = e.qref;
                    prev_tref = e.tref;
                    continue;
                }
            }
        }
        if constexpr (WAVE && !EXT) {
            if (sync_idx < n && sync_idx >= cbase) {
                const int l = int(sync_idx - cbase);
                const bool ns = cbase + lane_ < n && !(ccur.b >> 31) && ccur.qref >= query_var_pos && ccur.tref >= truth_var_pos;
                const unsigned long long below = (l == 63) ? ~0ull : ((2ull << l) - 1ull);
                const unsigned long long stop = ~__ballot(ns) & below;
                const int run = stop ? l - (63 - __builtin_clzll(stop)) : l + 1;
                if (run >= 2) {
                    const int lj = l - run + 1;
                    const unsigned long long in_run = below & ~((1ull << lj) - 1ull);
                    query_ed += __popcll(__ballot(ns && ((ccur.b >> 30) & 1u)) & in_run);
                    clean = false;
                    prev_qref = __builtin_amdgcn_readlane(ccur.qref, lj);
                    prev_tref = __builtin_amdgcn_readlane(ccur.tref, lj);
                    cur_b = uint32_t(__builtin_amdgcn_readlane(int(ccur.b), lj));
                    prev_hi = int(uint32_t(__builtin_amdgcn_readlane(int(ccur.a), lj)) >> 31);
                    prev_ti = int(cur_b & 0x0fffffffu);
                    eq_cur = (cur_b >> 28) & 3u;
                    sync_idx -= run;
                    if (sync_idx < 0) break;
                    cur_hi = prev_hi;
                    const PathEnt e = fetch(sync_idx);
                    cur_b = e.b;
                    eq_next = eq_cur; eq_cur = (e.b >> 28) & 3u;
                    nx_qref = prev_qref; nx_ti = prev_ti;
                    prev_qri = int(e.a & 0x7fffffffu);
                    prev_hi = int(e.a >> 31);
                    prev_ti = int(e.b & 0x0fffffffu);
                    prev_qref = e.qref;
                    prev_tref = e.tref;
                    continue;
                }
            }
        }
        const int query_ref_pos = prev_qref;
        while (query_ref_pos < query_var_pos && query_var_ptr >= d.qv_beg) {
            if (cur_hi == ri) {
                if (lead) fpg[query_var_ptr] = sync_group;
                sync_group++;
            }
            query_var_ptr--;
            query_var_pos = (query_var_ptr < d.qv_beg) ? -1 : qv_pos[query_var_ptr];
        }
        const int truth_ref_pos = prev_tref;
        while (truth_ref_pos < truth_var_pos && truth_var_ptr >= d.tv_beg) {
            truth_var_ptr--;
            truth_var_pos = (truth_var_ptr < d.tv_beg) ? -1 : tv_pos[truth_var_ptr];
        }
        const bool is_sync = (sync_idx == n) ? true : bool(cur_b >> 31);
        const int is_edit = (sync_idx == n) ? 0 : int((cur_b >> 30) & 1);
        if (is_sync) {
            const int sync_ref_idx = prev_qref + 1;
            const int sync_truth_idx = prev_ti + 1;
            int rl = prev_sync_ref_idx - sync_ref_idx, tl = prev_sync_truth_idx - sync_truth_idx;
            if (rl < 0 || rl > r_size - sync_ref_idx) rl = r_size - sync_ref_idx;
            if (tl < 0 || tl > t_size - sync_truth_idx) tl = t_size - sync_truth_idx;
            const bool has_q = query_var_ptr != prev_query_var_ptr;
            const bool has_t = truth_var_ptr != prev_truth_var_ptr;
            int ref_ed = -1;
            bool deferred = false;
            if (rl == 0) ref_ed = tl;
            else if (tl == 0) ref_ed = rl;
            else if (rl == 1 && tl == 1)
                ref_ed = ((eq_next & 2u) && nx_qref == sync_ref_idx && nx_ti == sync_truth_idx) ? int(!(eq_next & 1u))
                                                                                                : int(rs_at(sync_ref_idx) != ts_at(sync_truth_idx));
            else if (!has_q && !has_t && rl == tl) {
                bool same = true;
                for (int k = rl - 1; k >= 0 && same; k--) same = (rs_at(sync_ref_idx + k) == ts_at(sync_truth_idx + k));
                if (same) ref_ed = 0;
            }
            if (ref_ed < 0) {
                if (tl <= 32 && rl <= ED_INLINE_LONG) ref_ed = small_ed(Rs + sync_ref_idx, rl, Ts + sync_truth_idx, tl);
                else if (rl <= 32 && tl <= ED_INLINE_LONG) ref_ed = small_ed(Ts + sync_truth_idx, tl, Rs + sync_ref_idx, rl);
                else deferred = true;
            }
            if (has_q || has_t || deferred) {
                if (n_sec < d.sec_cap) {
                    Section S;
                    S.q_lo = int32_t(query_var_ptr); S.q_hi = int32_t(prev_query_var_ptr);
                    S.t_lo = int32_t(truth_var_ptr); S.t_hi = int32_t(prev_truth_var_ptr);
                    S.sync_group = sync_group; S.query_ed = query_ed; S.ref_ed = ref_ed;
                    S.flags = (deferred ? SEC_DEFERRED : 0) | ((has_q || has_t) ? 0 : SEC_NOVAR);
                    if (deferred && lead) {
                        const int32_t j = atomicAdd(n_jobs, 1);
                        if (j < jobs_cap) jobs[j] = EdJob{a, n_sec, sync_ref_idx, rl, sync_truth_idx, tl};
                        else status |= VPR_ST_ERR_LIMIT;
                    }
                    if (lead) sec[n_sec] = S;
                    n_sec++;
                } else status |= VPR_ST_ERR_LIMIT;
            } else {
                if (ref_ed != 0) status |= VPR_ST_WARN_REF_ED;
                if (query_ed != ref_ed) status |= VPR_ST_WARN_QUERY_ED;
                if (query_ed > ref_ed) status |= VPR_ST_WARN_EXCEEDS;
            }
            if (has_q || has_t) sync_group++;
            prev_query_var_ptr = query_var_ptr;
            prev_truth_var_ptr = truth_var_ptr;
            prev_sync_ref_idx = sync_ref_idx;
            prev_sync_truth_idx = sync_truth_idx;
            query_ed = 0;
        }
        query_ed += is_edit;
        clean = is_sync && !is_edit;
        sync_idx--;
        if (sync_idx < 0) break;
        cur_hi = prev_hi;
        const PathEnt e = fetch(sync_idx);
        cur_b = e.b;
        eq_next = eq_cur; eq_cur = (e.b >> 28) & 3u;
        nx_qref = prev_qref; nx_ti = prev_ti;
        prev_qri = int(e.a & 0x7fffffffu);
        prev_hi = int(e.a >> 31);
        prev_ti = int(e.b & 0x0fffffffu);
        prev_qref = e.qref;
        prev_tref = e.tref;
    }
    (void)prev_qri; (void)prev_ti;
    if (lead) {
        O.n_sec = n_sec;
        if (status) atomicOr(&O.status, status);
    }
}

#define WALK_TR 32
#define WALK_TW 256
template <bool WAVE>
__global__ void __launch_bounds__(64) k_walk(DevBatch B, const AlnDesc *__restrict__ descs,
                       const int32_t *__restrict__ work, int n_work,
                       const uint8_t *__restrict__ ws, const int32_t *__restrict__ blo_all,
                       AlnOut *__restrict__ outs,
                       PathEnt *__restrict__ paths, Section *__restrict__ secs,
                       int32_t *const *__restrict__ fp_group ,
                       EdJob *__restrict__ jobs, int32_t *__restrict__ n_jobs, int32_t jobs_cap, int my_w, int ok_tag) {
    __shared__ __align__(16) uint8_t tile[WAVE ? 2 * WALK_TR * WALK_TW : 16];
    __shared__ int32_t tblo[WAVE ? 2 * WALK_TR : 2];
    const int wi = WAVE ? int(blockIdx.x) : int(blockIdx.x * blockDim.x + threadIdx.x);
    if (wi >= n_work) return;
    if (WAVE) __builtin_amdgcn_s_setprio(2);
    const int lane = threadIdx.x & 63;
    const bool lead = !WAVE || lane == 0;
    const int a = work[wi];
    const AlnDesc d = descs[a];
    AlnOut &O = outs[a];
    if (d.band_pad != my_w || (my_w > 0 ? O.band_ok != ok_tag : O.band_ok < 0)) return;
    const int qi = 0, ri = 1;
    const int32_t *q2r = B.hap_ptr[d.qs] + d.q_off;
    const uint8_t *qfl = B.hap_flag[d.qs] + d.q_off;
    const int32_t *t2r = B.hap_ptr[d.ts] + d.t_off;
    const uint8_t *tfl = B.hap_flag[d.ts] + d.t_off;
    const int32_t *r2q = B.ref_ptr[d.qs] + d.r_off;
    const uint8_t *insQ = B.has_ins[d.qs] + d.r_off;
    const uint8_t *insT = B.has_ins[d.ts] + d.r_off;
    const uint8_t *mat[2] = {ws + d.mat_off[0], ws + d.mat_off[1]};
// ... 555 lines not shown
```

### vcfdist_amd/csrc/pr_zl.hip

```cpp
#ifndef PR_ZL_HIP_
#define PR_ZL_HIP_
#include <type_traits>


#define ZW_PTR(w) (int((w) & 0xffffu) - 1)
#define ZW_BASE(w) (((w) >> 16) & 0x7fu)
#define ZW_PV (1u << 23)
#define ZW_PB (1u << 24)
#define ZW_PE (1u << 25)
#define ZW_INS (1u << 26)
#define ZW_TP (1u << 27)
__device__ __forceinline__ bool zw_fwd_allow(uint32_t w) { return !(w & ZW_PV) || (w & ZW_PE); }
__device__ __forceinline__ bool zw_bwd_allow(uint32_t w) { return !(w & ZW_PV) || (w & ZW_PB); }

#define ZE_ALIVE 1u
#define ZE_HASMAT 2u
#define ZE_HASSWP 4u
#define ZE_PSLOT_SHIFT 3
#define ZE_TP 32u
#define ZE_BWD 64u

#define ZL_MAXLEN 65000
#define ZL_CLEAN_REJECT (-1)

__global__ void __launch_bounds__(256) k_prep_zl(DevBatch B, const AlnDesc *__restrict__ descs, const int32_t *__restrict__ list,
                                                 int n_list, const ZlWave *__restrict__ hdr, uint32_t *__restrict__ zin) {
    __shared__ uint32_t tile[64][65];
    __shared__ int64_t s_qo[64], s_ro[64], s_to[64];
    __shared__ int32_t s_lq[64], s_lr[64], s_lt[64];
    __shared__ uint8_t s_qs[64], s_ts[64];
    const int w = blockIdx.x;
    const ZlWave H = hdr[w];
    const int lane = threadIdx.x & 63, sub = threadIdx.x >> 6;
    if (threadIdx.x < 64) {
        const int wi = w * 64 + lane;
        const int a = wi < n_list ? list[wi] : -1;
        if (a >= 0) {
            const AlnDesc *d = descs + a;
            s_qo[lane] = d->q_off; s_ro[lane] = d->r_off; s_to[lane] = d->t_off;
            s_lq[lane] = d->Lq; s_lr[lane] = d->Lr; s_lt[lane] = d->Lt;
            s_qs[lane] = uint8_t(d->qs); s_ts[lane] = uint8_t(d->ts);
        } else {
            s_qo[lane] = s_ro[lane] = s_to[lane] = 0;
            s_lq[lane] = s_lr[lane] = s_lt[lane] = 0;
            s_qs[lane] = 0; s_ts[lane] = 2;
        }
    }
    __syncthreads();
    auto flagbits = [](int f) -> uint32_t { return ((f & PV) ? ZW_PV : 0u) | ((f & PB) ? ZW_PB : 0u) | ((f & PE) ? ZW_PE : 0u); };
    uint32_t *out = zin + H.in_off;
    for (int arr = 0; arr < 3; arr++) {
        const int mlen = arr == 0 ? H.mq : (arr == 1 ? H.mr : H.mt);
        for (int x0 = 0; x0 < mlen; x0 += 64) {
            const int x = x0 + lane;
#pragma unroll 16
            for (int k = 0; k < 16; k++) {
                const int l = sub * 16 + k;
                const int qs = s_qs[l], ts = s_ts[l];
                const int Lr = s_lr[l];
                const int len = arr == 0 ? s_lq[l] : (arr == 1 ? Lr : s_lt[l]);
                uint32_t v = 0x7f0000u;
                if (x < len) {
                    const int64_t ro = s_ro[l];
                    const int slot = arr == 2 ? ts : qs;
                    const int64_t o = (arr == 0 ? s_qo[l] : (arr == 1 ? ro : s_to[l])) + x;
                    const uint8_t *seq = arr == 1 ? B.ref_seq : B.hap_seq[slot];
                    const int2 *wk = arr == 0 ? B.wk_q[qs] : (arr == 1 ? B.wk_r[qs] : B.wk_t[ts - 2]);
                    const int2 k2 = wk[o];
                    const int p = k2.x, f = arr == 1 ? int(B.ref_flag[qs][o]) : (k2.y & 0xff);
                    const uint32_t ins = ((k2.y >> 8) & ((1 << qs) | (1 << ts))) ? ZW_INS : 0u;
                    v = uint32_t((p + 1) & 0xffff) | (uint32_t(seq[o] & 0x7f) << 16) | flagbits(f) | ins;
                    if (arr == 0 && x > 0 && ((p != wk[o - 1].x + 1) || (f & PB))) v |= ZW_TP;
                    (void)Lr;
                }
                tile[lane][l] = v;
            }
            __syncthreads();
            const int rows = min(64, mlen - x0);
            for (int r = sub; r < rows; r += 4) out[int64_t(x0 + r) * 64 + lane] = tile[r][lane];
            __syncthreads();
        }
        out += int64_t(mlen) * 64;
    }
}

typedef __attribute__((ext_vector_type(4))) unsigned int zl_u4;
typedef __attribute__((ext_vector_type(2))) unsigned int zl_u2;
#define ZL_OOB 0xfffffff0u

__global__ void __launch_bounds__(64, 6) k_zero_lane(const AlnDesc *__restrict__ descs, const int32_t *__restrict__ list, int n_list,
                                                  const ZlWave *__restrict__ hdr, const uint32_t *__restrict__ zin,
                                                  uint4 *__restrict__ zlog, AlnOut *__restrict__ outs, PathEnt *__restrict__ paths,
                                                  int keep_paths, int d1_max_rows, int prio_rows) {
    const int w = blockIdx.x, lane = threadIdx.x;
    const ZlWave H = hdr[w];
    if (H.mt >= prio_rows) __builtin_amdgcn_s_setprio(2);
    const int wi = w * 64 + lane;
    const int a_ = wi < n_list ? list[wi] : -1;
    const bool live = a_ >= 0;
    const int a = max(a_, 0);
    const AlnDesc *dp = descs + a;
    const int Lq = live ? dp->Lq : 1, Lr = live ? dp->Lr : 1, Lt = live ? dp->Lt : 0;
    const int L[2] = {Lq, Lr};
    const auto rin = __builtin_amdgcn_make_buffer_rsrc(const_cast<uint32_t *>(zin + H.in_off), 0, 256 * (H.mq + H.mr + H.mt), 0x00020000);
    const auto rlog = __builtin_amdgcn_make_buffer_rsrc(zlog + H.log_off, 0, 1280 * H.mt, 0x00020000);
    const uint32_t lane4 = uint32_t(lane) << 2, lane8 = uint32_t(lane) << 3;
    const uint32_t pos0[2] = {0u, uint32_t(H.mq) << 8}, post = uint32_t(H.mq + H.mr) << 8;
    const uint32_t logP0 = uint32_t(H.mt) << 9;
    auto in_at = [&](uint32_t off) -> uint32_t { return __builtin_amdgcn_raw_buffer_load_b32(rin, off, 0, 0); };
    bool ok = live && Lq < ZL_MAXLEN && Lr < ZL_MAXLEN && Lt < ZL_MAXLEN && Lt >= 2;
    const int rows = ok ? Lt : 0;
    int tmax = rows;
#pragma unroll
    for (int o = 32; o; o >>= 1) tmax = max(tmax, __shfl_xor(tmax, o));
    if (tmax == 0) {
        if (live) { outs[a].dist_q = D_INF; outs[a].dist_r = D_INF; outs[a].exit_min = 0; }
        return;
    }

    int qri[2][4];
    uint32_t pw[2][4];
#pragma unroll
    for (int p = 0; p < 2; p++) {
#pragma unroll
        for (int s = 0; s < 4; s++) { qri[p][s] = -1; pw[p][s] = 0; }
    }
    uint32_t tw0 = in_at(ok ? post + lane4 : ZL_OOB);
    if (ok) {
        qri[0][0] = 0; pw[0][0] = in_at(pos0[0] + lane4);
        qri[1][0] = 0; pw[1][0] = in_at(pos0[1] + lane4);
        zl_u2 e0;
        e0.x = ZE_ALIVE | ZE_HASMAT | ((pw[0][0] & ZW_TP) ? ZE_TP : 0u) | (zw_bwd_allow(pw[0][0]) ? ZE_BWD : 0u);
        e0.y = ZE_ALIVE | ZE_HASMAT | (zw_bwd_allow(pw[1][0]) ? ZE_BWD : 0u);
        __builtin_amdgcn_raw_buffer_store_b64(e0, rlog, lane8, 0, 0);
    }
    uint32_t pf_mw[2][2] = {{0, 0}, {0, 0}}, pf_sw[2][2] = {{0, 0}, {0, 0}};
    bool have_pf = false;
    auto fwd_row = [&](auto Sc, int t, bool act, uint32_t tw1) -> bool {
        constexpr int S = decltype(Sc)::value;
        const bool t_allow = zw_fwd_allow(tw0);
        uint32_t mw[2][S], sw[2][S];
        int sz[2][S];
        const bool use_pf = S == 2 && have_pf;
#pragma unroll
        for (int p = 0; p < 2; p++) {
#pragma unroll
            for (int s = 0; s < S; s++) {
                const bool alive = act && qri[p][s] >= 0;
                const int c = qri[p][s] + 1;
                const int z = ZW_PTR(pw[p][s]) + 1;
                const bool sok = alive && t_allow && zw_fwd_allow(pw[p][s]) && z < L[1 - p];
                sz[p][s] = sok ? z : -1;
                if (use_pf) {
                    mw[p][s] = (alive && c < L[p]) ? pf_mw[p][s & 1] : 0u;
                    sw[p][s] = sok ? pf_sw[p][s & 1] : 0u;
                } else {
                    mw[p][s] = in_at((alive && c < L[p]) ? pos0[p] + (uint32_t(c) << 8) + lane4 : ZL_OOB);
                    sw[p][s] = in_at(sok ? pos0[1 - p] + (uint32_t(z) << 8) + lane4 : ZL_OOB);
                }
            }
        }
        const uint32_t Tb = ZW_BASE(tw1);
        int nq[2][S];
        uint32_t nw[2][S], ne[2][S];
#pragma unroll
        for (int p = 0; p < 2; p++) {
#pragma unroll
            for (int s = 0; s < S; s++) {
                const bool hit = act && qri[p][s] >= 0 && ZW_BASE(mw[p][s]) == Tb;
                nq[p][s] = hit ? qri[p][s] + 1 : -1;
                nw[p][s] = mw[p][s];
                ne[p][s] = hit ? ZE_HASMAT : 0u;
            }
        }
        bool bad = false, full = false;
#pragma unroll
        for (int p = 0; p < 2; p++) {
            const int o = 1 - p;
#pragma unroll
            for (int s = 0; s < S; s++) {
                const bool hit = sz[p][s] >= 0 && ZW_BASE(sw[p][s]) == Tb;
                if (!__any(hit)) continue;
                const int z = sz[p][s];
                int at = -1;
#pragma unroll
                for (int k = S - 1; k >= 0; k--) at = (nq[o][k] < 0) ? k : at;
#pragma unroll
                for (int k = 0; k < S; k++) at = (nq[o][k] == z) ? k : at;
                full = full || (hit && at < 0);
#pragma unroll
                for (int k = 0; k < S; k++) {
                    const bool here = hit && at == k;
                    bad = bad || (here && (ne[o][k] & ZE_HASSWP));
                    nq[o][k] = here ? z : nq[o][k];
                    nw[o][k] = here ? sw[p][s] : nw[o][k];
                    ne[o][k] = here ? (ne[o][k] | ZE_HASSWP | (uint32_t(s) << ZE_PSLOT_SHIFT)) : ne[o][k];
                }
            }
        }
        if (S < 4 && __any(full)) return false;
        ok = ok && !bad && !full;
        if (S == 2) {
#pragma unroll
            for (int p = 0; p < 2; p++) {
#pragma unroll
                for (int s = 0; s < 2; s++) {
                    const bool alive = act && ok && nq[p][s] >= 0;
                    const int c = nq[p][s] + 1;
                    const int z = ZW_PTR(nw[p][s]) + 1;
                    pf_mw[p][s] = in_at((alive && c < L[p]) ? pos0[p] + (uint32_t(c) << 8) + lane4 : ZL_OOB);
                    pf_sw[p][s] = in_at((alive && zw_fwd_allow(nw[p][s]) && z < L[1 - p]) ? pos0[1 - p] + (uint32_t(z) << 8) + lane4 : ZL_OOB);
                }
            }
        }
        have_pf = S == 2;
        {
            zl_u2 ev;
            uint32_t wq = 0, wr_ = 0;
#pragma unroll
            for (int sl = 0; sl < S; sl++) {
                wq |= (nq[0][sl] < 0 ? 0u : (ZE_ALIVE | ne[0][sl] | ((nw[0][sl] & ZW_TP) ? ZE_TP : 0u) | (zw_bwd_allow(nw[0][sl]) ? ZE_BWD : 0u))) << (8 * sl);
                wr_ |= (nq[1][sl] < 0 ? 0u : (ZE_ALIVE | ne[1][sl] | (zw_bwd_allow(nw[1][sl]) ? ZE_BWD : 0u))) << (8 * sl);
            }
            ev.x = wq; ev.y = wr_;
            __builtin_amdgcn_raw_buffer_store_b64(ev, rlog, (act && ok) ? (uint32_t(t + 1) << 9) + lane8 : ZL_OOB, 0, 0);
        }
#pragma unroll
        for (int p = 0; p < 2; p++) {
#pragma unroll
            for (int s = 0; s < S; s++) { qri[p][s] = act ? nq[p][s] : qri[p][s]; pw[p][s] = act ? nw[p][s] : pw[p][s]; }
        }
        tw0 = act ? tw1 : tw0;
        return true;
    };
    for (int t = 0; t + 1 < tmax; t++) {
        const bool act = ok && t + 1 < rows;
        const uint32_t tw1 = in_at(act ? post + (uint32_t(t + 1) << 8) + lane4 : ZL_OOB);
        bool upper = false;
#pragma unroll
        for (int p = 0; p < 2; p++) upper = upper || (act && (qri[p][2] >= 0 || qri[p][3] >= 0));
        if (__any(upper) || !fwd_row(std::integral_constant<int, 2>{}, t, act, tw1))
            (void)fwd_row(std::integral_constant<int, 4>{}, t, act, tw1);
    }
    int endq = -1, endr = -1;
#pragma unroll
    for (int s = 0; s < 4; s++) {
        if (qri[0][s] == Lq - 1) endq = s;
        if (qri[1][s] == Lr - 1) endr = s;
    }
    const bool clean = ok && Lt <= d1_max_rows;
    ok = ok && (endq >= 0 || endr >= 0);
    if (live) {
        AlnOut &o = outs[a];
        o.dist_q = (ok && endq >= 0) ? 0 : D_INF;
        o.dist_r = (ok && endr >= 0) ? 0 : D_INF;
        o.exit_min = ok ? D_INF : (clean ? ZL_CLEAN_REJECT : 0);
    }
    if (!__any(ok)) return;

    const int nrow = ok ? Lt : 0;
    int sc[2][4];
#pragma unroll
    for (int p = 0; p < 2; p++) {
#pragma unroll
        for (int s = 0; s < 4; s++) sc[p][s] = -1;
    }
    int bmax = nrow;
#pragma unroll
    for (int o = 32; o; o >>= 1) bmax = max(bmax, __shfl_xor(bmax, o));
    auto log_row = [&](int t, bool on) -> zl_u2 {
        return __builtin_amdgcn_raw_buffer_load_b64(rlog, on ? (uint32_t(t) << 9) + lane8 : ZL_OOB, 0, 0);
    };
    zl_u2 cur = zl_u2{0, 0};
    auto bwd_row = [&](auto Sc, int t, bool act, zl_u2 pre) {
        constexpr int S = decltype(Sc)::value;
        int best[2][S];
        uint32_t pp[2][S];
#pragma unroll
        for (int p = 0; p < 2; p++) {
#pragma unroll
            for (int s = 0; s < S; s++) { best[p][s] = -1; pp[p][s] = 0; }
        }
#pragma unroll
        for (int p = 0; p < 2; p++) {
            const int o = 1 - p;
#pragma unroll
            for (int s = 0; s < S; s++) {
                const bool on = act && sc[p][s] >= 0;
                const uint32_t e = ((p ? cur.y : cur.x) >> (8 * s)) & 0xffu;
                const int tp = (e & ZE_TP) ? 1 : 0;
                {
                    const bool m = on && (e & ZE_HASMAT);
                    const int v = sc[p][s] + tp;
                    const bool gt = m && v > best[p][s], eq = m && v == best[p][s];
                    best[p][s] = gt ? v : best[p][s];
                    pp[p][s] = gt ? 1u : (eq ? (pp[p][s] | 1u) : pp[p][s]);
                }
                {
                    const bool m = on && (e & ZE_HASSWP) && (e & ZE_BWD);
                    const int v = sc[p][s] + (p == 1 ? 0 : tp);
                    const int ps = int((e >> ZE_PSLOT_SHIFT) & 3u);
                    const uint32_t mine = 2u | (uint32_t(s) << 2);
#pragma unroll
                    for (int k = 0; k < S; k++) {
                        const bool h_ = m && ps == k;
                        const bool gt = h_ && v > best[o][k], eq = h_ && v == best[o][k];
                        best[o][k] = gt ? v : best[o][k];
                        pp[o][k] = gt ? mine : (eq ? ((pp[o][k] & 1u) | mine) : pp[o][k]);
                    }
                }
            }
        }
        uint32_t ppw = 0;
#pragma unroll
        for (int p = 0; p < 2; p++) {
#pragma unroll
            for (int s = 0; s < 4; s++) {
                if (s < S) {
                    ppw |= (best[p][s] >= 0 ? pp[p][s] : 0u) << (4 * (p * 4 + s));
                    sc[p][s] = act ? best[p][s] : sc[p][s];
                } else {
                    sc[p][s] = act ? -1 : sc[p][s];
                }
            }
        }
        __builtin_amdgcn_raw_buffer_store_b32(ppw, rlog, act ? logP0 + (uint32_t(t - 1) << 8) + lane4 : ZL_OOB, 0, 0);
        if (act) cur = pre;
    };
    auto row_at = [&](int r) -> zl_u2 { return log_row(r, r >= 0 && r < nrow); };
    zl_u2 lastpre = row_at(bmax - 1);
    zl_u2 rA = row_at(bmax - 2), rB = row_at(bmax - 3), rC = row_at(bmax - 4), rD = zl_u2{0, 0};
    auto bwd_step = [&](int t, const zl_u2 &pre_reg, zl_u2 &next_reg) {
        const bool act = t >= 1 && t < nrow;
        const bool first = t == nrow - 1 && t >= 1;
        if (first) {
            const int ep = endq >= 0 ? 0 : 1, es = endq >= 0 ? endq : endr;
            cur = lastpre;
#pragma unroll
            for (int p = 0; p < 2; p++) {
#pragma unroll
                for (int s = 0; s < 4; s++) sc[p][s] = (p == ep && s == es) ? 0 : -1;
            }
        }
        next_reg = row_at(t - 4);
        const zl_u2 pre = pre_reg;
        const bool upper = act && (((cur.x | cur.y | pre.x | pre.y) & 0xffff0000u) != 0u);
        if (__any(upper)) bwd_row(std::integral_constant<int, 4>{}, t, act, pre);
        else bwd_row(std::integral_constant<int, 2>{}, t, act, pre);
        lastpre = pre;
    };
    for (int t = bmax - 1; t >= 1; t -= 4) {
        bwd_step(t, rA, rD);
        bwd_step(t - 1, rB, rA);
        bwd_step(t - 2, rC, rB);
        bwd_step(t - 3, rD, rC);
    }
    const int beg_plane = sc[0][0] >= 0 ? VPR_PLANE_QUERY : VPR_PLANE_REF;

    if (ok) outs[a].beg_plane = beg_plane;
}

__global__ void __launch_bounds__(64, 8) k_zero_walk(const AlnDesc *__restrict__ descs, const int32_t *__restrict__ list, int n_list,
                                                  const ZlWave *__restrict__ hdr, const uint32_t *__restrict__ zin,
                                                  uint4 *__restrict__ zlog, AlnOut *__restrict__ outs, PathEnt *__restrict__ paths,
                                                  int keep_paths, int tag, int prio_rows) {
    const int w = blockIdx.x, lane = threadIdx.x;
    const ZlWave H = hdr[w];
    if (H.mt >= prio_rows) __builtin_amdgcn_s_setprio(2);
    const int wi = w * 64 + lane;
    const int a_ = wi < n_list ? list[wi] : -1;
    const bool live = a_ >= 0;
    const int a = max(a_, 0);
    const AlnDesc *dp = descs + a;
    const auto rin = __builtin_amdgcn_make_buffer_rsrc(const_cast<uint32_t *>(zin + H.in_off), 0, 256 * (H.mq + H.mr + H.mt), 0x00020000);
    const auto rlog = __builtin_amdgcn_make_buffer_rsrc(zlog + H.log_off, 0, 1280 * H.mt, 0x00020000);
    const uint32_t lane4 = uint32_t(lane) << 2, lane8 = uint32_t(lane) << 3;
    const uint32_t pos0[2] = {0u, uint32_t(H.mq) << 8}, post = uint32_t(H.mq + H.mr) << 8;
    const uint32_t logP0 = uint32_t(H.mt) << 9, logS0 = logP0 + (uint32_t(H.mt) << 8);
    auto in_at = [&](uint32_t off) -> uint32_t { return __builtin_amdgcn_raw_buffer_load_b32(rin, off, 0, 0); };
    const bool ok = live && dp->band_pad == tag && outs[a].band_ok == tag;
    const int nrow = ok ? dp->Lt : 0;
    int bmax = nrow;
#pragma unroll
    for (int o = 32; o; o >>= 1) bmax = max(bmax, __shfl_xor(bmax, o));
    if (bmax == 0) return;
    const int beg_plane = ok ? outs[a].beg_plane : 0;
    PathEnt *path = paths + dp->path_off;
    int hi = beg_plane, slot = 0, mv_in = 0, x = 0;
    uint32_t status = 0;
    bool wok = ok;
    for (int t = 0; t < bmax; t++) {
        const bool act = wok && t < nrow;
        const uint32_t ppw = __builtin_amdgcn_raw_buffer_load_b32(rlog, (act && t + 1 < nrow) ? logP0 + (uint32_t(t) << 8) + lane4 : ZL_OOB, 0, 0);
        const uint32_t tw = in_at(act ? post + (uint32_t(t) << 8) + lane4 : ZL_OOB);
        const uint32_t cw = in_at(act ? pos0[hi] + (uint32_t(x) << 8) + lane4 : ZL_OOB);
        const int trv = ZW_PTR(tw), qref = hi ? x : ZW_PTR(cw);
        uint32_t sync = 1;
        if (mv_in) {
            const bool in_t = (tw & ZW_PV) && !(tw & ZW_PB);
            const bool in_q = hi == 0 && (cw & ZW_PV) && !(cw & ZW_PB);
            sync = (!in_t && !in_q && !((tw | cw) & ZW_INS) && trv == qref) ? 1u : 0u;
        }
        const uint32_t eqb = (ZW_BASE(cw) == ZW_BASE(tw) ? 1u : 0u) | ((hi || !(cw & ZW_PV)) ? 2u : 0u);
        zl_u2 st;
        st.x = uint32_t(x) | (uint32_t(hi) << 16) | (sync << 17) | (eqb << 18);
        st.y = uint32_t(qref + 1) | (uint32_t(trv + 1) << 16);
        __builtin_amdgcn_raw_buffer_store_b64(st, rlog, act ? logS0 + (uint32_t(t) << 9) + lane8 : ZL_OOB, 0, 0);
        if ((keep_paths & 1) && act) {
            uint4 pe;
            pe.x = uint32_t(x) | (uint32_t(hi) << 31);
            pe.y = uint32_t(t) | (sync << 31);
            pe.z = uint32_t(qref);
            pe.w = uint32_t(trv);
            *reinterpret_cast<uint4 *>(path + t) = pe;
        }
        if (act && t + 1 < nrow) {
            const uint32_t nb = (ppw >> (4 * ((hi << 2) | slot))) & 15u;
            if (hi == 1 && (nb & 2u)) { hi = 0; slot = int(nb >> 2); x = ZW_PTR(cw) + 1; }
            else if (nb & 1u) { x = x + 1; }
            else if (hi == 0 && (nb & 2u)) { hi = 1; slot = int(nb >> 2); x = ZW_PTR(cw) + 1; }
            else { status |= VPR_ST_ERR_NO_PTR; wok = false; }
            mv_in = 1;
        }
    }
    if (ok) {
        AlnOut &o = outs[a];
        o.path_len = wok ? nrow : 0;
        if (!wok) o.n_sec = 0;
        if (status) atomicOr(&o.status, status);
    }
}

struct ZlFetch {
    const uint2 *log;
    int64_t pre_i;
    uint2 pre;
    __device__ PathEnt operator()(int64_t i) {
        const uint2 v = (i == pre_i) ? pre : log[i * 64];
        if (i > 0) { pre_i = i - 1; pre = log[(i - 1) * 64]; }
        PathEnt e;
        e.a = (v.x & 0xffffu) | (((v.x >> 16) & 1u) << 31);
        e.b = uint32_t(i) | (((v.x >> 17) & 1u) << 31) | (((v.x >> 18) & 3u) << 28);
        e.qref = int(v.y & 0xffffu) - 1;
        e.tref = int(v.y >> 16) - 1;
        return e;
    }
};

__global__ void __launch_bounds__(64) k_zero_credit(DevBatch B, const AlnDesc *__restrict__ descs, const int32_t *__restrict__ list,
                                                    int n_list, const ZlWave *__restrict__ hdr, const uint4 *__restrict__ zlog,
                                                    AlnOut *__restrict__ outs, Section *__restrict__ secs,
                                                    int32_t *const *__restrict__ fp_group, EdJob *__restrict__ jobs,
                                                    int32_t *__restrict__ n_jobs, int32_t jobs_cap, int tag) {
    const int w = blockIdx.x, lane = threadIdx.x;
    const int wi = w * 64 + lane;
    if (wi >= n_list) return;
    const int a = list[wi];
    if (a < 0) return;
    const AlnDesc d = descs[a];
    AlnOut &O = outs[a];
    if (d.band_pad != tag || O.band_ok != tag) return;
    if (O.status & (VPR_ST_ERR_NO_PTR | VPR_ST_ERR_LIMIT)) return;
    const ZlWave H = hdr[w];
    ZlFetch f{reinterpret_cast<const uint2 *>(zlog + H.log_off + 48 * int64_t(H.mt)) + lane, -1, make_uint2(0, 0)};
    credit_walk<false, ZlFetch, true>(B, d, O, a, nullptr, int64_t(O.path_len), 0u, secs, fp_group, jobs, n_jobs, jobs_cap, true, f);
}

#endif
```

Baseline: 202.0 million supercluster-alignments/s.

## Fuse credit walk into zero/one-distance lane walk kernels, drop path log

The credit pass is merged into k_zero_walk and k_one_walk. A forward FwdCredit state machine now consumes each path step as it is produced, one step behind. This replaces the separate k_zero_credit and k_one_credit kernels, which re-read a stored per-step path log backwards. The per-row path log region is removed, so the log stride shrinks from 80 to 48 words per row and the memory estimates change to match. The risks are higher register pressure in the walk kernels, extra per-step branching and a reference-base load, and possible divergence in the forward credit logic from the old backward walk.

Result: no change. 200.3 million supercluster-alignments/s (-0.8%).

```diff
diff --git a/vcfdist_amd/csrc/pr_api.hip b/vcfdist_amd/csrc/pr_api.hip
--- a/vcfdist_amd/csrc/pr_api.hip
+++ b/vcfdist_amd/csrc/pr_api.hip
@@ -117,7 +117,7 @@
     int lm = 0;
     for (int k = b; k < e; k++) {
         const ZlWave W = hdr[k];
-        si += 64 * (int64_t(W.mq) + W.mr + W.mt); sl += 80 * int64_t(W.mt);
+        si += 64 * (int64_t(W.mq) + W.mr + W.mt); sl += 48 * int64_t(W.mt);
         lm = max(lm, max(W.mq, max(W.mr, W.mt)));
     }
     s_in[tid] = si; s_log[tid] = sl;
@@ -132,7 +132,7 @@
     for (int k = b; k < e; k++) {
         ZlWave W = hdr[k];
         W.in_off = oi; W.log_off = ol;
-        oi += 64 * (int64_t(W.mq) + W.mr + W.mt); ol += 80 * int64_t(W.mt);
+        oi += 64 * (int64_t(W.mq) + W.mr + W.mt); ol += 48 * int64_t(W.mt);
         hdr[k] = W;
     }
     if (lm) atomicMax(&s_len, lm);
@@ -737,7 +737,7 @@
             W.in_off = in_words;
             W.log_off = log_cur;
             in_words += 64 * (int64_t(W.mq) + W.mr + W.mt);
-            log_cur += 80 * int64_t(W.mt);
+            log_cur += 48 * int64_t(W.mt);
             len_max = std::max(len_max, std::max(W.mq, std::max(W.mr, W.mt)));
         }
         log_max = std::max(log_max, log_cur);
@@ -760,7 +760,7 @@
         const double D1_SHARE = 0.4;
         const int64_t D1_FLOOR = int64_t(4) << 20;
         const int64_t slack = 64 * 5 * int64_t(len_max + 1);
-        const int64_t in_all = 2 * in_chunk_max + slack, log_all = 2 * log_max + 160 * int64_t((n_short_max + 63) / 64) + 160 * int64_t(len_max + 1);
+        const int64_t in_all = 2 * in_chunk_max + slack, log_all = log_max / 48 * 160 + 160 * int64_t((n_short_max + 63) / 64) + 160 * int64_t(len_max + 1);
         h->d1_in_cap = std::min(in_all, std::max(int64_t(D1_SHARE * double(in_all)), D1_FLOOR + slack));
         h->d1_log_cap = std::min(log_all, std::max(int64_t(D1_SHARE * double(log_all)), D1_FLOOR + slack));
         const int64_t cap_ip = std::min<int64_t>(n_short_max, std::max<int64_t>(4096, (n_short_max / 4 + 3) & ~int64_t(3)));
@@ -1386,8 +1386,9 @@
     avail = std::max<int64_t>(avail - h->mem_reserve, avail / 2);
     int64_t lane_est = 0;
     if (h->p0.valid && h->cfg.band_mode != 0 && h->cfg.band_mode != 2) {
-        const double zl = 1.15 * (double(h->p0.part_in[1]) / 6.0 * 4.0 + 20.0 * double(h->p0.part_rows[1]));
-        lane_est = int64_t(zl * (getenv("VPR_NO_D1") ? 1.0 : 1.8)) + 28 * int64_t(h->descs.size());
+        const double zl_in = double(h->p0.part_in[1]) / 6.0 * 4.0, zl_rows = double(h->p0.part_rows[1]);
+        const double zl = 1.15 * (zl_in + 12.0 * zl_rows + (getenv("VPR_NO_D1") ? 0.0 : 0.8 * (zl_in + 20.0 * zl_rows)));
+        lane_est = int64_t(zl) + 28 * int64_t(h->descs.size());
         avail = std::max<int64_t>(avail - lane_est, avail / 2);
     }
     int64_t budget = h->cfg.workspace_bytes > 0 ? h->cfg.workspace_bytes : int64_t(double(avail) * arena_share());
@@ -2226,20 +2227,14 @@
             if (rc) return rc;
             ws_.cells_per_thread = 3;
             if (zero) {
-                ws_.bytes_algorithmic = 20 * zl_rows;
+                ws_.bytes_algorithmic = 12 * zl_rows;
                 rc = timed(3, ws_, ks, "k_zero_walk", [&] {
-                    hipLaunchKernelGGL(k_zero_walk, dim3((cnt + 63) / 64), dim3(64), 0, ks, h->d_descs, list, cnt, h->d_zl_hdr + zl_wave0,
+                    hipLaunchKernelGGL(k_zero_walk, dim3((cnt + 63) / 64), dim3(64), 0, ks, h->dB, h->d_descs, list, cnt, h->d_zl_hdr + zl_wave0,
                                        h->d_zl_in, h->d_zl_log, h->d_outs, a_path, (h->cfg.flags & VPR_CFG_KEEP_PATHS) ? 1 : 0, tag,
-                                       h->lane_prio_rows);
+                                       h->lane_prio_rows, FwdCreditOut{h->d_secs, {h->d_fp[0], h->d_fp[1], h->d_fp[2], h->d_fp[3]}, h->d_jobs, h->d_njobs, h->jobs_cap});
                 });
-                if (rc) return rc;
                 ws_.bytes_algorithmic = 0;
             }
-            if (zero) rc = timed(3, ws_, ks, "k_zero_credit", [&] {
-                hipLaunchKernelGGL(k_zero_credit, dim3((cnt + 63) / 64), dim3(64), 0, ks, h->dB, h->d_descs, list, cnt,
-                                   h->d_zl_hdr + zl_wave0, h->d_zl_log, h->d_outs, h->d_secs, h->d_fp_table, h->d_jobs,
-                                   h->d_njobs, h->jobs_cap, tag);
-            });
             else if (cnt <= CREDIT_WAVE_MAX && !n_dev) rc = timed(3, ws_, ks, "k_credit<wave>", [&] {
                 hipLaunchKernelGGL(k_credit<true>, dim3(cnt), dim3(64), 0, ks, h->dB, h->d_descs, list, cnt,
                                    h->d_outs, a_path, h->d_secs, h->d_fp_table, h->d_jobs, h->d_njobs,
@@ -2360,14 +2355,10 @@
         } else if (ph == 4) {
             ls.cells_per_thread = 3;
             rc = timed(3, ls, ks, "k_one_walk", [&] {
-                hipLaunchKernelGGL(k_one_walk, dim3(nw), dim3(64), 0, ks, h->d_descs, list, n_dev, cap, h->d_d1_hdr, h->d_d1_in, h->d_d1_log,
+                hipLaunchKernelGGL(k_one_walk, dim3(nw), dim3(64), 0, ks, h->dB, h->d_descs, list, n_dev, cap, h->d_d1_hdr, h->d_d1_in, h->d_d1_log,
                                    h->d_outs, reinterpret_cast<PathEnt *>(h->plan0.arena), (h->cfg.flags & VPR_CFG_KEEP_PATHS) ? 1 : 0, h->d_d1_info,
-                                   std::max(1, h->lane_prio_rows / 4));
-            });
-            if (rc) return rc;
-            rc = timed(3, ls, ks, "k_one_credit", [&] {
-                hipLaunchKernelGGL(k_one_credit, dim3(nw), dim3(64), 0, ks, h->dB, h->d_descs, list, n_dev, cap, h->d_d1_hdr, h->d_d1_log,
-                                   h->d_outs, h->d_secs, h->d_fp_table, h->d_jobs, h->d_njobs, h->jobs_cap, ztag);
+                                   std::max(1, h->lane_prio_rows / 4), ztag,
+                                   FwdCreditOut{h->d_secs, {h->d_fp[0], h->d_fp[1], h->d_fp[2], h->d_fp[3]}, h->d_jobs, h->d_njobs, h->jobs_cap});
             });
         }
         return rc;
diff --git a/vcfdist_amd/csrc/pr_d1.hip b/vcfdist_amd/csrc/pr_d1.hip
--- a/vcfdist_amd/csrc/pr_d1.hip
+++ b/vcfdist_amd/csrc/pr_d1.hip
@@ -628,11 +628,11 @@
     if (ok) { AlnOut &o = outs[a]; o.beg_plane = beg_plane; o.path_len = -1; }
 }
 
-__global__ void __launch_bounds__(64, 8) k_one_walk(const AlnDesc *__restrict__ descs, const int32_t *__restrict__ list,
+__global__ void __launch_bounds__(64, 8) k_one_walk(DevBatch B, const AlnDesc *__restrict__ descs, const int32_t *__restrict__ list,
                                                     const int32_t *__restrict__ n_dev, int n_cap, const ZlWave *__restrict__ hdr,
                                                     const uint32_t *__restrict__ zin, uint4 *__restrict__ zlog,
                                                     AlnOut *__restrict__ outs, PathEnt *__restrict__ paths, int keep_paths,
-                                                    int32_t *__restrict__ info, int prio_rows) {
+                                                    int32_t *__restrict__ info, int prio_rows, int ztag, FwdCreditOut co) {
     const int w = blockIdx.x, lane = threadIdx.x;
     const ZlWave H = hdr[w];
     if (H.mt <= 0) return;
@@ -652,28 +652,32 @@
     if (bmax == 0) return;
     const auto rin = __builtin_amdgcn_make_buffer_rsrc(const_cast<uint32_t *>(zin + H.in_off), 0, 256 * (2 * H.mq + 2 * H.mr + H.mt), 0x00020000);
     const auto rlog = __builtin_amdgcn_make_buffer_rsrc(zlog + H.log_off, 0, 2560 * (H.mt + 1), 0x00020000);
-    const uint32_t lane4 = uint32_t(lane) << 2, lane8 = uint32_t(lane) << 3, lane16 = uint32_t(lane) << 4;
+    const uint32_t lane4 = uint32_t(lane) << 2, lane16 = uint32_t(lane) << 4;
     const uint32_t posW[2] = {0u, uint32_t(2 * H.mq) << 8};
     const uint32_t post = uint32_t(2 * H.mq + 2 * H.mr) << 8;
-    const uint32_t logB1 = uint32_t(H.mt + 1) << 10;
     auto in_at = [&](uint32_t off) -> uint32_t { return __builtin_amdgcn_raw_buffer_load_b32(rin, off, 0, 0); };
     auto word_at = [&](int p, int x, bool on) -> uint32_t { return in_at(on ? posW[p] + (uint32_t(x) << 8) + lane4 : ZL_OOB); };
     auto t_at = [&](int t, bool on) -> uint32_t { return in_at(on ? post + (uint32_t(t) << 8) + lane4 : ZL_OOB); };
     const int beg_plane = ok ? outs[a].beg_plane : 0;
+    const bool credit = ok && dp->band_pad == ztag && !(outs[a].status & (VPR_ST_ERR_NO_PTR | VPR_ST_ERR_LIMIT));
+    FwdCredit<false> fc;
+    fc.init(B, dp, credit);
     auto lapck = [&](int) {};
     {
         PathEnt *path = paths + dp->path_off;
-        const uint32_t logS0 = logB1;
         int hi = beg_plane, slot = 0, layer = 0, x = 0, ti = 0, mv_in = -1;
         uint32_t status = 0;
         bool wok = ok, done = !ok;
         int plen = 0;
-        for (int i = 0; i <= bmax; i++) {
+        uint2 pe = make_uint2(0, 0);
+        uint32_t prw = 0;
+        for (int i = 0; i <= bmax + 1; i++) {
             const bool act = wok && !done;
-            if (!__any(act)) break;
+            if (!__any(act || (pe.x & FC_PEND))) break;
             const uint32_t mvw = __builtin_amdgcn_raw_buffer_load_b32(rlog, act ? (uint32_t(ti) << 10) + lane16 + (uint32_t(layer) << 3) + (uint32_t(hi) << 2) : ZL_OOB, 0, 0);
             const uint32_t tw = t_at(ti, act);
             const uint32_t cw = word_at(hi, x, act);
+            fc.step(B, co, dp, a, pe, int(pe.x >> FC_TI_SHIFT), prw);
             const int trv = ZW_PTR(tw), qref = hi ? x : ZW_PTR(cw);
             uint32_t sync = 1, edit = 0;
             if (mv_in >= 0) {
@@ -684,10 +688,10 @@
                 edit = (mv_in == MV_SUB || mv_in == MV_INS || mv_in == MV_DEL) ? 1u : 0u;
             }
             const uint32_t eqb = (ZW_BASE(cw) == ZW_BASE(tw) ? 1u : 0u) | ((hi || !(cw & ZW_PV)) ? 2u : 0u);
-            zl_u2 st;
-            st.x = uint32_t(x) | (uint32_t(hi) << 16) | (sync << 17) | (eqb << 18) | (edit << 20) | (uint32_t(i - ti) << 21);
-            st.y = uint32_t(qref + 1) | (uint32_t(trv + 1) << 16);
-            __builtin_amdgcn_raw_buffer_store_b64(st, rlog, act ? logS0 + (uint32_t(i) << 9) + lane8 : ZL_OOB, 0, 0);
+            const bool fin = act && layer == 1 && hi == 0 && x == Lq - 1 && ti == nrow - 1;
+            pe.x = fc_entry(act && credit, hi, sync, eqb, fin, i == 0, edit, tw, ti, qref, trv, pe.y);
+            pe.y = uint32_t(qref + 1) | (uint32_t(trv + 1) << 16);
+            prw = word_at(1, qref, FwdCredit<false>::wants_ref(pe.x));
             if ((keep_paths & 1) && act) {
                 uint4 pe;
                 pe.x = uint32_t(x) | (uint32_t(hi) << 31);
@@ -697,7 +701,7 @@
                 *reinterpret_cast<uint4 *>(path + i) = pe;
             }
             if (act) {
-                if (layer == 1 && hi == 0 && x == Lq - 1 && ti == nrow - 1) { done = true; plen = i + 1; }
+                if (fin) { done = true; plen = i + 1; }
                 else {
                     const uint32_t m = (mvw >> (8 * slot)) & 0xffu;
                     const int rank = int(m & 7u), to = int((m >> 3) & 3u);
@@ -723,46 +727,11 @@
             if (!wok) status |= VPR_ST_ERR_NO_PTR;
             o.beg_plane = beg_plane;
             o.path_len = wok ? plen : 0;
-            if (!wok) o.n_sec = 0;
+            if (credit) { fc.finish(co, dp, wok); status |= fc.status; }
+            if (credit || !wok) o.n_sec = wok ? fc.n_sec : 0;
             if (status) atomicOr(&o.status, status);
         }
     }
 }
 
-struct D1Fetch {
-    const uint2 *log;
-    int64_t pre_i;
-    uint2 pre;
-    __device__ PathEnt operator()(int64_t i) {
-        const uint2 v = (i == pre_i) ? pre : log[i * 64];
-        if (i > 0) { pre_i = i - 1; pre = log[(i - 1) * 64]; }
-        PathEnt e;
-        e.a = (v.x & 0xffffu) | (((v.x >> 16) & 1u) << 31);
-        e.b = uint32_t(i - int64_t((v.x >> 21) & 1u)) | (((v.x >> 17) & 1u) << 31) | (((v.x >> 20) & 1u) << 30) | (((v.x >> 18) & 3u) << 28);
-        e.qref = int(v.y & 0xffffu) - 1;
-        e.tref = int(v.y >> 16) - 1;
-        return e;
-    }
-};
-
-__global__ void __launch_bounds__(64) k_one_credit(DevBatch B, const AlnDesc *__restrict__ descs, const int32_t *__restrict__ list,
-                                                   const int32_t *__restrict__ n_dev, int n_cap, const ZlWave *__restrict__ hdr,
-                                                   const uint4 *__restrict__ zlog, AlnOut *__restrict__ outs, Section *__restrict__ secs,
-                                                   int32_t *const *__restrict__ fp_group, EdJob *__restrict__ jobs,
-                                                   int32_t *__restrict__ n_jobs, int32_t jobs_cap, int ztag) {
-    const int w = blockIdx.x, lane = threadIdx.x;
-    const ZlWave H = hdr[w];
-    if (H.mt <= 0) return;
-    const int wi = w * 64 + lane;
-    if (wi >= min(*n_dev, n_cap)) return;
-    const int a = list[wi];
-    if (a < 0) return;
-    const AlnDesc d = descs[a];
-    AlnOut &O = outs[a];
-    if (d.band_pad != ztag || O.band_ok != D1_TAG) return;
-    if (O.status & (VPR_ST_ERR_NO_PTR | VPR_ST_ERR_LIMIT)) return;
-    D1Fetch f{reinterpret_cast<const uint2 *>(zlog + H.log_off + 64 * (int64_t(H.mt) + 1)) + lane, -1, make_uint2(0, 0)};
-    credit_walk<false, D1Fetch, true>(B, d, O, a, nullptr, int64_t(O.path_len), 0u, secs, fp_group, jobs, n_jobs, jobs_cap, true, f);
-}
-
 #endif
diff --git a/vcfdist_amd/csrc/pr_kernels.hip b/vcfdist_amd/csrc/pr_kernels.hip
--- a/vcfdist_amd/csrc/pr_kernels.hip
+++ b/vcfdist_amd/csrc/pr_kernels.hip
@@ -563,13 +563,12 @@
     return row[n];
 }
 
-struct NoFetch { __device__ PathEnt operator()(int64_t) const { return PathEnt{0, 0, 0, 0}; } };
-template <bool WAVE, class XF = NoFetch, bool EXT = false>
+template <bool WAVE>
 __device__ __forceinline__ void credit_walk(const DevBatch &B, const AlnDesc &d, AlnOut &O, const int a,
                                             const PathEnt *__restrict__ path, const int64_t n, uint32_t status,
                                             Section *__restrict__ secs, int32_t *const *__restrict__ fp_group,
                                             EdJob *__restrict__ jobs, int32_t *__restrict__ n_jobs, int32_t jobs_cap,
-                                            const bool lead, XF xf = XF()) {
+                                            const bool lead) {
     const int qi = 0, ri = 1;
     const int32_t *q2r = B.hap_ptr[d.qs] + d.q_off;
     const int32_t *t2r = B.hap_ptr[d.ts] + d.t_off;
@@ -610,9 +609,7 @@
     PathEnt q0 = ccur, q1 = ccur, q2 = ccur, q3 = ccur, q4 = ccur, q5 = ccur, q6 = ccur, q7 = ccur;
     int64_t qbase = int64_t(1) << 60;
     auto fetch = [&](int64_t i) -> PathEnt {
-        if constexpr (EXT) {
-            return xf(i);
-        } else if (WAVE) {
+        if (WAVE) {
             if (i < cbase) {
                 cbase -= 64;
                 ccur = cpre;
@@ -695,7 +692,7 @@
         pl_base = cbase;
     };
     while (sync_idx >= 0) {
-        if constexpr (WAVE && !EXT) {
+        if constexpr (WAVE) {
             if (clean && sync_idx < n) {
                 if (pl_base != cbase) plain_static();
                 const int l = int(sync_idx - cbase);
@@ -729,7 +726,7 @@
                 }
             }
         }
-        if constexpr (WAVE && !EXT) {
+        if constexpr (WAVE) {
             if (sync_idx < n && sync_idx >= cbase) {
                 const int l = int(sync_idx - cbase);
                 const bool ns = cbase + lane_ < n && !(ccur.b >> 31) && ccur.qref >= query_var_pos && ccur.tref >= truth_var_pos;
diff --git a/vcfdist_amd/csrc/pr_zl.hip b/vcfdist_amd/csrc/pr_zl.hip
--- a/vcfdist_amd/csrc/pr_zl.hip
+++ b/vcfdist_amd/csrc/pr_zl.hip
@@ -1,5 +1,6 @@
 #ifndef PR_ZL_HIP_
 #define PR_ZL_HIP_
+#include <climits>
 #include <type_traits>
 
 
@@ -103,7 +104,7 @@
     const int Lq = live ? dp->Lq : 1, Lr = live ? dp->Lr : 1, Lt = live ? dp->Lt : 0;
     const int L[2] = {Lq, Lr};
     const auto rin = __builtin_amdgcn_make_buffer_rsrc(const_cast<uint32_t *>(zin + H.in_off), 0, 256 * (H.mq + H.mr + H.mt), 0x00020000);
-    const auto rlog = __builtin_amdgcn_make_buffer_rsrc(zlog + H.log_off, 0, 1280 * H.mt, 0x00020000);
+    const auto rlog = __builtin_amdgcn_make_buffer_rsrc(zlog + H.log_off, 0, 768 * H.mt, 0x00020000);
     const uint32_t lane4 = uint32_t(lane) << 2, lane8 = uint32_t(lane) << 3;
     const uint32_t pos0[2] = {0u, uint32_t(H.mq) << 8}, post = uint32_t(H.mq + H.mr) << 8;
     const uint32_t logP0 = uint32_t(H.mt) << 9;
@@ -360,10 +361,180 @@
     if (ok) outs[a].beg_plane = beg_plane;
 }
 
-__global__ void __launch_bounds__(64, 8) k_zero_walk(const AlnDesc *__restrict__ descs, const int32_t *__restrict__ list, int n_list,
+__device__ __noinline__ int small_ed_far(const uint8_t *a, int m, const uint8_t *b, int n) { return small_ed(a, m, b, n); }
+
+struct FwdCreditOut {
+    Section *secs;
+    int32_t *fp[4];
+    EdJob *jobs;
+    int32_t *n_jobs;
+    int32_t jobs_cap;
+};
+
+#define FC_HI 1u
+#define FC_SYNC 2u
+#define FC_EQ_SHIFT 2
+#define FC_LAST 16u
+#define FC_FIRST 32u
+#define FC_PEND 64u
+#define FC_BACK 128u
+#define FC_EDIT 256u
+#define FC_TBASE_SHIFT 9
+#define FC_TI_SHIFT 16
+__device__ __forceinline__ uint32_t fc_entry(bool on, int hi, uint32_t sync, uint32_t eqb, bool last, bool first, uint32_t edit,
+                                             uint32_t tw, int ti, int qref, int trv, uint32_t prev_y) {
+    const bool back = !first && (uint32_t(qref + 1) < (prev_y & 0xffffu) || uint32_t(trv + 1) < (prev_y >> 16));
+    return !on ? 0u : (hi ? FC_HI : 0u) | (sync ? FC_SYNC : 0u) | (eqb << FC_EQ_SHIFT) | (last ? FC_LAST : 0u) | (first ? FC_FIRST : 0u) |
+                      FC_PEND | (back ? FC_BACK : 0u) | (edit ? FC_EDIT : 0u) | (ZW_BASE(tw) << FC_TBASE_SHIFT) | (uint32_t(ti) << FC_TI_SHIFT);
+}
+
+template <bool DIAG>
+struct FwdCredit {
+    int open_q, open_t;
+    int nq0, nq1, nt0, nt1;
+    int qp, tp, qv_end, tv_end;
+    int sec_q0, sec_t0;
+    int base, nfp, qed, n_sec;
+    int sec_cap;
+    int64_t sec_off;
+    uint32_t status;
+    int aln;
+    bool any_fp, bad;
+
+    __device__ __forceinline__ const int32_t *qv(const DevBatch &B) const { return (aln & 2) ? B.var_pos[1] : B.var_pos[0]; }
+    __device__ __forceinline__ const int32_t *tv(const DevBatch &B) const { return (aln & 1) ? B.var_pos[3] : B.var_pos[2]; }
+    __device__ __forceinline__ int32_t *fpg(const FwdCreditOut &o) const {
+        return aln == 0 ? o.fp[0] : (aln == 1 ? o.fp[1] : (aln == 2 ? o.fp[3] : o.fp[2]));
+    }
+
+    __device__ __forceinline__ void init(const DevBatch &B, const AlnDesc *dp, bool on) {
+        aln = dp->aln & 3;
+        qp = int(dp->qv_beg); tp = int(dp->tv_beg);
+        qv_end = on ? int(dp->qv_end) : qp; tv_end = on ? int(dp->tv_end) : tp;
+        sec_off = dp->sec_off; sec_cap = dp->sec_cap;
+        const int32_t *q = qv(B), *t = tv(B);
+        nq0 = qp < qv_end ? q[qp] : INT_MAX; nq1 = qp + 1 < qv_end ? q[qp + 1] : INT_MAX;
+        nt0 = tp < tv_end ? t[tp] : INT_MAX; nt1 = tp + 1 < tv_end ? t[tp + 1] : INT_MAX;
+        open_q = open_t = 0;
+        sec_q0 = qp; sec_t0 = tp;
+        base = nfp = qed = n_sec = 0;
+        status = 0;
+        any_fp = bad = false;
+    }
+    __device__ __forceinline__ void pop_q(const DevBatch &B, const FwdCreditOut &o, int lim, bool mark) {
+        while (qp < qv_end && nq0 <= lim) {
+            if (mark) { fpg(o)[qp] = -2 - (base + 1 + nfp); nfp++; any_fp = true; }
+            qp++;
+            nq0 = nq1;
+            nq1 = qp + 1 < qv_end ? qv(B)[qp + 1] : INT_MAX;
+        }
+    }
+    __device__ __forceinline__ void pop_t(const DevBatch &B, int lim) {
+        while (tp < tv_end && nt0 <= lim) {
+            tp++;
+            nt0 = nt1;
+            nt1 = tp + 1 < tv_end ? tv(B)[tp + 1] : INT_MAX;
+        }
+    }
+    __device__ __forceinline__ void close(const DevBatch &B, const FwdCreditOut &o, const AlnDesc *dp, int a, int rl, int tl, bool one_ne) {
+        const int sref = open_q + 1, stru = open_t + 1;
+        const bool has_q = qp != sec_q0, has_t = tp != sec_t0;
+        const int qe = DIAG ? 0 : qed;
+        int ref_ed = -1;
+        bool deferred = false;
+        if (rl == 0) ref_ed = tl;
+        else if (tl == 0) ref_ed = rl;
+        else if (rl == 1 && tl == 1) ref_ed = int(one_ne);
+        else {
+            const uint8_t *Rs = B.ref_seq + dp->r_off + sref;
+            const uint8_t *Ts = ((aln & 1) ? B.hap_seq[3] : B.hap_seq[2]) + dp->t_off + stru;
+            if (!has_q && !has_t && rl == tl) {
+                bool same = true;
+                for (int k = rl - 1; k >= 0 && same; k--) same = Rs[k] == Ts[k];
+                if (same) ref_ed = 0;
+            }
+            if (ref_ed < 0) {
+                if (tl <= 32 && rl <= ED_INLINE_LONG) ref_ed = small_ed_far(Rs, rl, Ts, tl);
+                else if (rl <= 32 && tl <= ED_INLINE_LONG) ref_ed = small_ed_far(Ts, tl, Rs, rl);
+                else deferred = true;
+            }
+        }
+        if (has_q || has_t || deferred) {
+            if (n_sec < sec_cap) {
+                Section S;
+                S.q_lo = sec_q0 - 1; S.q_hi = qp - 1; S.t_lo = sec_t0 - 1; S.t_hi = tp - 1;
+                S.sync_group = base; S.query_ed = qe; S.ref_ed = ref_ed;
+                S.flags = (deferred ? SEC_DEFERRED : 0) | ((has_q || has_t) ? 0 : SEC_NOVAR);
+                if (deferred) {
+                    const int32_t j = atomicAdd(o.n_jobs, 1);
+                    if (j < o.jobs_cap) o.jobs[j] = EdJob{a, n_sec, sref, rl, stru, tl};
+                    else status |= VPR_ST_ERR_LIMIT;
+                }
+                o.secs[sec_off + n_sec] = S;
+                n_sec++;
+            } else status |= VPR_ST_ERR_LIMIT;
+        } else {
+            if (ref_ed != 0) status |= VPR_ST_WARN_REF_ED;
+            if (qe != ref_ed) status |= VPR_ST_WARN_QUERY_ED;
+            if (qe > ref_ed) status |= VPR_ST_WARN_EXCEEDS;
+        }
+        base += ((has_q || has_t) ? 1 : 0) + nfp;
+        nfp = 0; qed = 0;
+        sec_q0 = qp; sec_t0 = tp;
+    }
+    __device__ __forceinline__ void step(const DevBatch &B, const FwdCreditOut &o, const AlnDesc *dp, int a, uint2 e, int ti, uint32_t rw) {
+        if (!(e.x & FC_PEND)) return;
+        const int qref = int(e.y & 0xffffu) - 1, trv = int(e.y >> 16) - 1;
+        const bool hi = e.x & FC_HI, last = e.x & FC_LAST;
+        if (e.x & FC_FIRST) {
+            pop_q(B, o, qref, false);
+            pop_t(B, trv);
+            sec_q0 = qp; sec_t0 = tp;
+            open_q = qref; open_t = ti;
+            return;
+        }
+        bad = bad || (e.x & FC_BACK);
+        if (!DIAG) qed += (e.x & FC_EDIT) ? 1 : 0;
+        if (qref >= nq0) pop_q(B, o, qref, hi);
+        if (trv >= nt0) pop_t(B, trv);
+        if ((e.x & FC_SYNC) || last) {
+            const int rl = qref - open_q, tl = ti - open_t;
+            const uint32_t eq = (e.x >> FC_EQ_SHIFT) & 3u;
+            const bool plain = rl == 1 && tl == 1 && eq == 3u && (DIAG || qed == 0) && qp == sec_q0 && tp == sec_t0;
+            if (!plain && !bad)
+                close(B, o, dp, a, rl, tl, (eq & 2u) ? !(eq & 1u) : ZW_BASE(rw) != ((e.x >> FC_TBASE_SHIFT) & 0x7fu));
+            open_q = qref; open_t = ti;
+        }
+        if (last && !bad) {
+            pop_q(B, o, INT_MAX, hi);
+            pop_t(B, INT_MAX);
+            close(B, o, dp, a, dp->Lr - (qref + 1), dp->Lt - (ti + 1), false);
+        }
+    }
+    static __device__ __forceinline__ bool wants_ref(uint32_t ex) { return (ex & FC_PEND) && (ex & (FC_SYNC | FC_LAST)) && !((ex >> FC_EQ_SHIFT) & 2u); }
+    __device__ __forceinline__ void finish(const FwdCreditOut &o, const AlnDesc *dp, bool walked) {
+        const bool good = walked && !bad;
+        if (!good) n_sec = 0;
+        if (walked && bad) status |= VPR_ST_ERR_LIMIT;
+        const int total = base;
+        for (int k = 0; k < n_sec; k++) {
+            int32_t *g = &o.secs[sec_off + k].sync_group;
+            *g = total - 1 - *g;
+        }
+        if (any_fp) {
+            int32_t *f = fpg(o);
+            for (int v = int(dp->qv_beg); v < qp; v++) {
+                const int32_t g = f[v];
+                if (g <= -2) f[v] = good ? total - 1 - (-2 - g) : -1;
+            }
+        }
+    }
+};
+
+__global__ void __launch_bounds__(64, 8) k_zero_walk(DevBatch B, const AlnDesc *__restrict__ descs, const int32_t *__restrict__ list, int n_list,
                                                   const ZlWave *__restrict__ hdr, const uint32_t *__restrict__ zin,
                                                   uint4 *__restrict__ zlog, AlnOut *__restrict__ outs, PathEnt *__restrict__ paths,
-                                                  int keep_paths, int tag, int prio_rows) {
+                                                  int keep_paths, int tag, int prio_rows, FwdCreditOut co) {
     const int w = blockIdx.x, lane = threadIdx.x;
     const ZlWave H = hdr[w];
     if (H.mt >= prio_rows) __builtin_amdgcn_s_setprio(2);
@@ -373,10 +544,10 @@
     const int a = max(a_, 0);
     const AlnDesc *dp = descs + a;
     const auto rin = __builtin_amdgcn_make_buffer_rsrc(const_cast<uint32_t *>(zin + H.in_off), 0, 256 * (H.mq + H.mr + H.mt), 0x00020000);
-    const auto rlog = __builtin_amdgcn_make_buffer_rsrc(zlog + H.log_off, 0, 1280 * H.mt, 0x00020000);
-    const uint32_t lane4 = uint32_t(lane) << 2, lane8 = uint32_t(lane) << 3;
+    const auto rlog = __builtin_amdgcn_make_buffer_rsrc(zlog + H.log_off, 0, 768 * H.mt, 0x00020000);
+    const uint32_t lane4 = uint32_t(lane) << 2;
     const uint32_t pos0[2] = {0u, uint32_t(H.mq) << 8}, post = uint32_t(H.mq + H.mr) << 8;
-    const uint32_t logP0 = uint32_t(H.mt) << 9, logS0 = logP0 + (uint32_t(H.mt) << 8);
+    const uint32_t logP0 = uint32_t(H.mt) << 9;
     auto in_at = [&](uint32_t off) -> uint32_t { return __builtin_amdgcn_raw_buffer_load_b32(rin, off, 0, 0); };
     const bool ok = live && dp->band_pad == tag && outs[a].band_ok == tag;
     const int nrow = ok ? dp->Lt : 0;
@@ -385,15 +556,20 @@
     for (int o = 32; o; o >>= 1) bmax = max(bmax, __shfl_xor(bmax, o));
     if (bmax == 0) return;
     const int beg_plane = ok ? outs[a].beg_plane : 0;
-    PathEnt *path = paths + dp->path_off;
+    const bool credit = ok && !(outs[a].status & (VPR_ST_ERR_NO_PTR | VPR_ST_ERR_LIMIT));
+    FwdCredit<true> fc;
+    fc.init(B, dp, credit);
     int hi = beg_plane, slot = 0, mv_in = 0, x = 0;
     uint32_t status = 0;
     bool wok = ok;
-    for (int t = 0; t < bmax; t++) {
+    uint2 pe = make_uint2(0, 0);
+    uint32_t prw = 0;
+    for (int t = 0; t <= bmax; t++) {
         const bool act = wok && t < nrow;
         const uint32_t ppw = __builtin_amdgcn_raw_buffer_load_b32(rlog, (act && t + 1 < nrow) ? logP0 + (uint32_t(t) << 8) + lane4 : ZL_OOB, 0, 0);
         const uint32_t tw = in_at(act ? post + (uint32_t(t) << 8) + lane4 : ZL_OOB);
         const uint32_t cw = in_at(act ? pos0[hi] + (uint32_t(x) << 8) + lane4 : ZL_OOB);
+        fc.step(B, co, dp, a, pe, t - 1, prw);
         const int trv = ZW_PTR(tw), qref = hi ? x : ZW_PTR(cw);
         uint32_t sync = 1;
         if (mv_in) {
@@ -402,11 +578,11 @@
             sync = (!in_t && !in_q && !((tw | cw) & ZW_INS) && trv == qref) ? 1u : 0u;
         }
         const uint32_t eqb = (ZW_BASE(cw) == ZW_BASE(tw) ? 1u : 0u) | ((hi || !(cw & ZW_PV)) ? 2u : 0u);
-        zl_u2 st;
-        st.x = uint32_t(x) | (uint32_t(hi) << 16) | (sync << 17) | (eqb << 18);
-        st.y = uint32_t(qref + 1) | (uint32_t(trv + 1) << 16);
-        __builtin_amdgcn_raw_buffer_store_b64(st, rlog, act ? logS0 + (uint32_t(t) << 9) + lane8 : ZL_OOB, 0, 0);
+        pe.x = fc_entry(act && credit, hi, sync, eqb, t + 1 == nrow, t == 0, 0u, tw, 0, qref, trv, pe.y);
+        pe.y = uint32_t(qref + 1) | (uint32_t(trv + 1) << 16);
+        prw = in_at(FwdCredit<true>::wants_ref(pe.x) ? pos0[1] + (uint32_t(qref) << 8) + lane4 : ZL_OOB);
         if ((keep_paths & 1) && act) {
+            PathEnt *path = paths + dp->path_off;
             uint4 pe;
             pe.x = uint32_t(x) | (uint32_t(hi) << 31);
             pe.y = uint32_t(t) | (sync << 31);
@@ -426,44 +602,10 @@
     if (ok) {
         AlnOut &o = outs[a];
         o.path_len = wok ? nrow : 0;
-        if (!wok) o.n_sec = 0;
+        if (credit) { fc.finish(co, dp, wok); status |= fc.status; }
+        if (credit || !wok) o.n_sec = wok ? fc.n_sec : 0;
         if (status) atomicOr(&o.status, status);
     }
 }
 
-struct ZlFetch {
-    const uint2 *log;
-    int64_t pre_i;
-    uint2 pre;
-    __device__ PathEnt operator()(int64_t i) {
-        const uint2 v = (i == pre_i) ? pre : log[i * 64];
-        if (i > 0) { pre_i = i - 1; pre = log[(i - 1) * 64]; }
-        PathEnt e;
-        e.a = (v.x & 0xffffu) | (((v.x >> 16) & 1u) << 31);
-        e.b = uint32_t(i) | (((v.x >> 17) & 1u) << 31) | (((v.x >> 18) & 3u) << 28);
-        e.qref = int(v.y & 0xffffu) - 1;
-        e.tref = int(v.y >> 16) - 1;
-        return e;
-    }
-};
-
-__global__ void __launch_bounds__(64) k_zero_credit(DevBatch B, const AlnDesc *__restrict__ descs, const int32_t *__restrict__ list,
-                                                    int n_list, const ZlWave *__restrict__ hdr, const uint4 *__restrict__ zlog,
-                                                    AlnOut *__restrict__ outs, Section *__restrict__ secs,
-                                                    int32_t *const *__restrict__ fp_group, EdJob *__restrict__ jobs,
-                                                    int32_t *__restrict__ n_jobs, int32_t jobs_cap, int tag) {
-    const int w = blockIdx.x, lane = threadIdx.x;
-    const int wi = w * 64 + lane;
-    if (wi >= n_list) return;
-    const int a = list[wi];
-    if (a < 0) return;
-    const AlnDesc d = descs[a];
-    AlnOut &O = outs[a];
-    if (d.band_pad != tag || O.band_ok != tag) return;
-    if (O.status & (VPR_ST_ERR_NO_PTR | VPR_ST_ERR_LIMIT)) return;
-    const ZlWave H = hdr[w];
-    ZlFetch f{reinterpret_cast<const uint2 *>(zlog + H.log_off + 48 * int64_t(H.mt)) + lane, -1, make_uint2(0, 0)};
-    credit_walk<false, ZlFetch, true>(B, d, O, a, nullptr, int64_t(O.path_len), 0u, secs, fp_group, jobs, n_jobs, jobs_cap, true, f);
-}
-
 #endif
```
